# remit0/SpeechRecognitionProject

Hardware: AMD Instinct MI355X
Metric: utterances/sec (1 s @16 kHz) MFCC+CNN-BiGRU train step (higher is better)
Workload: dtype fp32; 1 GPU; cfg2 mfcc_bgru: on-device MFCC[39x51] + 2-layer BiGRU(512) + FC, CE, backward, Adam (full training.py step), per-GPU batch 256; model=mfcc_bgru, global_batch=256, clip_samples=16000, parallelism=dp1, step_execution=HIP graph replay of the whole step, sync_bn=False

## Files before the change

include/srk.h:

```cpp
#ifndef SRK_H_
#define SRK_H_

#include <stdint.h>

#define SRK_ABI_VERSION 3

#ifdef __cplusplus
extern "C" {
#endif

enum srk_status {
  SRK_OK = 0,
  SRK_ERR_INVALID = -1,
  SRK_ERR_HIP = -2,
  SRK_ERR_INTERNAL = -3,
  SRK_ERR_TIMEOUT = -4,
};

int srk_version(void);
const char* srk_source_stamp(void);
const char* srk_last_error(void);
int srk_init(int device);
int64_t srk_scratch_generation(void);
int srk_prof_enable(int on);
// ... 24 lines not shown
                  const int64_t* file_idx, const int64_t* offset, const double* gain,
                  int64_t n_clips, float* out, void* stream);

int srk_spec_noise_fwd(const int16_t* pcm, const int16_t* bank, int64_t n_files, int64_t bank_len,
                       const int64_t* file_idx, const int64_t* offset, const double* gain, int64_t n_clips,
                       float* out, int transposed, void* stream);

int srk_softmax_ensemble(const float* logits, int64_t K, int64_t B, int64_t C, float* probs_cat, float* mean,
                         int64_t* pred, void* stream);

enum { SRK_WAV_ERR_OPEN = -1, SRK_WAV_ERR_FORMAT = -2, SRK_WAV_ERR_UNSUPPORTED = -3 };
int srk_wav_read_batch(const char* const* paths, int64_t n, int16_t* out, int64_t* lengths, int n_threads);

enum { SRK_AUG_NONE = 0, SRK_AUG_SPEED = 1, SRK_AUG_SHIFT = 2, SRK_AUG_NOISE = 3, SRK_AUG_NOISE_SNR = 4,
       SRK_AUG_SILENCE = 5, SRK_AUG_PITCH = 6  };
int srk_augment(const int16_t* pcm, int64_t n_clips, const int16_t* bank, int64_t bank_len, const int32_t* op,
                const int64_t* iparam, const int64_t* noise_pos, const double* dparam, uint64_t seed, float* out,
                void* stream);

int64_t srk_pitch_workspace_bytes(int64_t n_shift);
int srk_pitch_shift(const int16_t* pcm, int64_t n_clips, const int32_t* clip_idx, const int32_t* level_idx,
                    int64_t n_shift, float* out, void* workspace, int64_t workspace_bytes, void* stream);

int srk_gemm_f32(int trans_a, int trans_b, int64_t M, int64_t N, int64_t K, float alpha, const float* A,
                 int64_t lda, const float* B, int64_t ldb, float beta, float* C, int64_t ldc,
                 const float* bias, int bias_mode, void* stream);
int srk_gemm_rowsum_f32(int trans_a, int trans_b, int64_t M, int64_t N, int64_t K, float alpha, const float* A,
                        int64_t lda, const float* B, int64_t ldb, float beta, float* C, int64_t ldc,
                        float* rowsum, void* stream);
int srk_gemm_16(int trans_a, int trans_b, int64_t M, int64_t N, int64_t K, float alpha, const uint16_t* A,
                int64_t lda, const uint16_t* B, int64_t ldb, float beta, float* C, int64_t ldc,
                const float* bias, int bias_mode, void* stream);
int srk_gemm_16_batched(int trans_a, int trans_b, int64_t M, int64_t N, int64_t K, float alpha,
                        const uint16_t* A, int64_t lda, int64_t sA, const uint16_t* B, int64_t ldb,
                        int64_t sB, float beta, float* C, int64_t ldc, int64_t sC, int batch, void* stream);
int srk_colsum_f32(const float* X, int64_t M, int64_t N, int64_t ldx, float* out, float beta, void* stream);

int64_t srk_gru_workspace_floats(int64_t B, int64_t T, int64_t in, int64_t H, int backward);
int srk_gru_layer_fwd(const float* x, int64_t B, int64_t T, int64_t in, int64_t H, const float* w_ih,
                      const float* w_hh, const float* b_ih, const float* b_hh, float* y, float* ws,
                      void* stream);
int srk_gru_layer_bwd(const float* x, int64_t B, int64_t T, int64_t in, int64_t H, const float* w_ih,
                      const float* w_hh, const float* y, const float* ws_fwd, const float* dy, float* dx,
                      float* dw_ih, float* dw_hh, float* db_ih, float* db_hh, int accumulate, float* ws,
                      void* stream);
int64_t srk_gru_y16_offset(int64_t B, int64_t T, int64_t in, int64_t H);
int srk_gru_layer_fwd_x16(const float* x, const void* x16, int64_t B, int64_t T, int64_t in, int64_t H,
                          const float* w_ih, const float* w_hh, const float* b_ih, const float* b_hh, float* y,
                          float* ws, void* stream);
int srk_gru_layer_bwd_x16(const float* x, const void* x16, int64_t B, int64_t T, int64_t in, int64_t H,
                          const float* w_ih, const float* w_hh, const float* y, const float* ws_fwd, const float* dy,
                          float* dx, float* dw_ih, float* dw_hh, float* db_ih, float* db_hh, int accumulate,
                          float* ws, void* stream);

int64_t srk_conv2d_workspace_floats(int64_t Ci, int64_t Co, int64_t KH, int64_t KW);
int srk_conv2d_nhwc_fwd(const float* x, int64_t N, int64_t H, int64_t W, int64_t Ci, const float* w,
                        const float* bias, int64_t Co, int64_t KH, int64_t KW, int64_t ph, int64_t pw, int64_t sh,
                        int64_t sw, float* y, float* ws, void* stream);
int srk_conv2d_nhwc_bwd(const float* x, int64_t N, int64_t H, int64_t W, int64_t Ci, const float* w, int64_t Co,
                        int64_t KH, int64_t KW, int64_t ph, int64_t pw, int64_t sh, int64_t sw, const float* dy,
                        float* dx, float* dw, float* db, float* ws, void* stream);
int srk_conv2d_nhwc_fwd16(const float* x, int64_t N, int64_t H, int64_t W, int64_t Ci, const float* w,
                          const float* bias, int64_t Co, int64_t KH, int64_t KW, int64_t ph, int64_t pw, int64_t sh,
                          int64_t sw, float* y, float* ws, void* x16, int* x16_written, void* stream);
int srk_conv2d_nhwc_bwd16(const float* x, int64_t N, int64_t H, int64_t W, int64_t Ci, const float* w, int64_t Co,
                          int64_t KH, int64_t KW, int64_t ph, int64_t pw, int64_t sh, int64_t sw, const float* dy,
                          float* dx, float* dw, float* db, float* ws, const void* x16, void* stream);
int srk_conv2d_nhwc_bwd16_dy16(const float* x, int64_t N, int64_t H, int64_t W, int64_t Ci, const float* w,
                               int64_t Co, int64_t KH, int64_t KW, int64_t ph, int64_t pw, int64_t sh, int64_t sw,
                               const float* dy, const void* dy16, float* dx, float* dw, float* db, float* ws,
                               const void* x16, void* stream);
int srk_conv2d_nhwc_bwd16_acc(const float* x, int64_t N, int64_t H, int64_t W, int64_t Ci, const float* w,
                              int64_t Co, int64_t KH, int64_t KW, int64_t ph, int64_t pw, int64_t sh, int64_t sw,
                              const float* dy, const void* dy16, float* dx, float* dw, float* db, float* ws,
                              const void* x16, int dw_accumulate, void* stream);
int srk_conv1d_nlc_dil_fwd(const float* x, int64_t N, int64_t L, int64_t Ci, const float* w, const float* bias,
                           int64_t Co, int64_t K, int64_t pad, int64_t dil, float* y, float* ws,
                           void* x16, int* x16_written, void* stream);
int srk_conv1d_nlc_dil_bwd(const float* x, int64_t N, int64_t L, int64_t Ci, const float* w, int64_t Co, int64_t K,
                           int64_t pad, int64_t dil, const float* dy, const void* dy16, float* dx, float* dw,
                           float* db, float* ws, const void* x16, int dw_accumulate, void* stream);
int srk_conv2d_nhwc_fwd_pool(const float* x, int64_t N, int64_t H, int64_t W, int64_t Ci, const float* w,
                             const float* bias, int64_t Co, int64_t KH, int64_t KW, int64_t ph, int64_t pw,
                             int64_t pool_w, float* y, uint8_t* argmax, float* ws, void* x16, int* x16_written,
                             void* stream);
int srk_conv2d_nhwc_bwd_pool(const float* x, int64_t N, int64_t H, int64_t W, int64_t Ci, const float* w, int64_t Co,
                             int64_t KH, int64_t KW, int64_t ph, int64_t pw, int64_t pool_w, const float* dy_pooled,
                             const uint8_t* argmax, float* dx, float* dw, float* db, float* ws, const void* x16,
                             void* stream);
int64_t srk_conv1_pool_workspace_floats(int64_t Co, int64_t KH, int64_t KW);
int srk_conv1_pool_fwd(const float* x, int64_t N, int64_t H, int64_t W, const float* w, const float* bias,
                       int64_t Co, int64_t KH, int64_t KW, int64_t ph, int64_t pw, int64_t pool, float* y,
                       uint8_t* argmax, void* stream);
int srk_conv1_pool_fwd16(const float* x, int64_t N, int64_t H, int64_t W, const float* w, const float* bias,
                         int64_t Co, int64_t KH, int64_t KW, int64_t ph, int64_t pw, int64_t pool, float* y,
                         uint8_t* argmax, void* y16, int* y16_written, void* stream);
int srk_conv1_pool_wgrad(const float* x, int64_t N, int64_t H, int64_t W, int64_t Co, int64_t KH, int64_t KW,
                         int64_t ph, int64_t pw, int64_t pool, const float* dy, const uint8_t* argmax, float* dw,
                         float* db, float* ws, void* stream);
int srk_conv1_pool_dgrad(const float* w, int64_t N, int64_t H, int64_t W, int64_t Co, int64_t KH, int64_t KW,
                         int64_t ph, int64_t pw, int64_t pool, const float* dy, const uint8_t* argmax, float* dx,
                         void* stream);
int srk_maxpool_nhwc_fwd(const float* x, int64_t N, int64_t H, int64_t W, int64_t C, int64_t kh, int64_t kw,
                         float* y, void* stream);
int srk_maxpool_nhwc_bwd(const float* x, const float* dy, int64_t N, int64_t H, int64_t W, int64_t C, int64_t kh,
                         int64_t kw, float* dx, void* stream);
// ... 88 lines not shown
```

speechrecognitionproject_amd/_lib.py:

```python
import ctypes
import os
import re

import torch

_HERE = os.path.dirname(os.path.abspath(__file__))
LIB_PATH = os.environ.get("SRK_LIB") or os.path.join(_HERE, "libsrk.so")
HEADER = os.path.join(os.path.dirname(_HERE), "include", "srk.h")
ABI_VERSION = 3

_P = ctypes.c_void_p
_I64 = ctypes.c_int64
_I = ctypes.c_int
_F = ctypes.c_float
_D = ctypes.c_double

_SIGS = {
    "srk_version": [],
    "srk_last_error": [],
    "srk_init": [_I],
    "srk_prof_enable": [_I],
    "srk_prof_read": [ctypes.c_char_p, ctypes.POINTER(ctypes.c_int64), ctypes.POINTER(ctypes.c_double),
                      ctypes.POINTER(ctypes.c_double)],
    "srk_prof_kernels": [ctypes.c_char_p, _I64, ctypes.POINTER(ctypes.c_int64)],
    "srk_source_stamp": [],
    "srk_diag_acc_store": [_P, _I64, _I, _P],
    "srk_diag_tr16_read": [_P, _I64, _P, _P],
    "srk_set_option": [ctypes.c_char_p, _I64],
    "srk_spin_timeouts": [],
    "srk_scratch_generation": [],
    "srk_gru_audit_words": [_I64, _I, _I, ctypes.POINTER(ctypes.c_int64), ctypes.POINTER(ctypes.c_int64),
                            ctypes.POINTER(ctypes.c_int64)],
    "srk_health_check": [_I],
    "srk_health_reset": [],
    "srk_fbank_fwd": [_P, _I64, _P, _P],
    "srk_mfcc_fwd": [_P, _I64, _P, _I, _P],
    "srk_spec_fwd": [_P, _I64, _P, _I, _P],
    "srk_fbank_fwd_i16": [_P, _I64, _P, _P],
    "srk_mfcc_fwd_i16": [_P, _I64, _P, _I, _P],
    "srk_spec_fwd_i16": [_P, _I64, _P, _I, _P],
    "srk_fbank_vtlp_fwd": [_P, _I64, _P, _P, _P],
    "srk_fbank_vtlp_fwd_i16": [_P, _I64, _P, _P, _P],
    "srk_vtlp_bins": [_D, ctypes.POINTER(ctypes.c_int32)],
    "srk_uniform_f64_state": [_P, _D, _D, _I64, _P, _P],
    "srk_noise_mix": [_P, _P, _I64, _I64, _P, _P, _P, _I64, _P, _P],
    "srk_spec_noise_fwd": [_P, _P, _I64, _I64, _P, _P, _P, _I64, _P, _I, _P],
    "srk_augment": [_P, _I64, _P, _I64, _P, _P, _P, _P, ctypes.c_uint64, _P, _P],
    "srk_pitch_workspace_bytes": [_I64],
    "srk_pitch_shift": [_P, _I64, _P, _P, _I64, _P, _P, _I64, _P],
    "srk_wav_read_batch": [ctypes.POINTER(ctypes.c_char_p), _I64, _P, _P, _I],
    "srk_softmax_ensemble": [_P, _I64, _I64, _I64, _P, _P, _P, _P],
    "srk_gemm_f32": [_I, _I, _I64, _I64, _I64, _F, _P, _I64, _P, _I64, _F, _P, _I64, _P, _I, _P],
    "srk_gemm_rowsum_f32": [_I, _I, _I64, _I64, _I64, _F, _P, _I64, _P, _I64, _F, _P, _I64, _P, _P],
    "srk_gemm_16": [_I, _I, _I64, _I64, _I64, _F, _P, _I64, _P, _I64, _F, _P, _I64, _P, _I, _P],
    "srk_gemm_16_batched": [_I, _I, _I64, _I64, _I64, _F, _P, _I64, _I64, _P, _I64, _I64, _F, _P, _I64, _I64, _I, _P],
    "srk_colsum_f32": [_P, _I64, _I64, _I64, _P, _F, _P],
    "srk_gru_workspace_floats": [_I64, _I64, _I64, _I64, _I],
    "srk_gru_layer_fwd": [_P, _I64, _I64, _I64, _I64, _P, _P, _P, _P, _P, _P, _P],
    "srk_gru_layer_bwd": [_P, _I64, _I64, _I64, _I64, _P, _P, _P, _P, _P, _P, _P, _P, _P, _P, _I, _P, _P],
    "srk_gru_y16_offset": [_I64, _I64, _I64, _I64],
    "srk_gru_layer_fwd_x16": [_P, _P, _I64, _I64, _I64, _I64, _P, _P, _P, _P, _P, _P, _P],
    "srk_gru_layer_bwd_x16": [_P, _P, _I64, _I64, _I64, _I64, _P, _P, _P, _P, _P, _P, _P, _P, _P, _P, _I, _P, _P],
    "srk_conv2d_workspace_floats": [_I64, _I64, _I64, _I64],
    "srk_conv2d_nhwc_fwd": [_P, _I64, _I64, _I64, _I64, _P, _P, _I64, _I64, _I64, _I64, _I64, _I64, _I64, _P, _P,
                            _P],
    "srk_conv2d_nhwc_bwd": [_P, _I64, _I64, _I64, _I64, _P, _I64, _I64, _I64, _I64, _I64, _I64, _I64, _P, _P, _P,
                            _P, _P, _P],
    "srk_conv2d_nhwc_fwd16": [_P, _I64, _I64, _I64, _I64, _P, _P, _I64, _I64, _I64, _I64, _I64, _I64, _I64, _P, _P,
                              _P, ctypes.POINTER(_I), _P],
    "srk_conv2d_nhwc_bwd16": [_P, _I64, _I64, _I64, _I64, _P, _I64, _I64, _I64, _I64, _I64, _I64, _I64, _P, _P, _P,
                              _P, _P, _P, _P],
    "srk_conv2d_nhwc_bwd16_dy16": [_P, _I64, _I64, _I64, _I64, _P, _I64, _I64, _I64, _I64, _I64, _I64, _I64, _P, _P,
                                   _P, _P, _P, _P, _P, _P],
    "srk_conv2d_nhwc_bwd16_acc": [_P, _I64, _I64, _I64, _I64, _P, _I64, _I64, _I64, _I64, _I64, _I64, _I64, _P, _P,
                                  _P, _P, _P, _P, _P, _I, _P],
    "srk_conv1d_nlc_dil_fwd": [_P, _I64, _I64, _I64, _P, _P, _I64, _I64, _I64, _I64, _P, _P, _P, ctypes.POINTER(_I), _P],
    "srk_conv1d_nlc_dil_bwd": [_P, _I64, _I64, _I64, _P, _I64, _I64, _I64, _I64, _P, _P, _P, _P, _P, _P, _P, _I, _P],
    "srk_conv2d_nhwc_fwd_pool": [_P, _I64, _I64, _I64, _I64, _P, _P, _I64, _I64, _I64, _I64, _I64, _I64, _P, _P, _P,
                                 _P, ctypes.POINTER(_I), _P],
    "srk_conv2d_nhwc_bwd_pool": [_P, _I64, _I64, _I64, _I64, _P, _I64, _I64, _I64, _I64, _I64, _I64, _P, _P, _P, _P,
                                 _P, _P, _P, _P],
    "srk_conv1_pool_workspace_floats": [_I64, _I64, _I64],
    "srk_conv1_pool_fwd": [_P, _I64, _I64, _I64, _P, _P, _I64, _I64, _I64, _I64, _I64, _I64, _P, _P, _P],
    "srk_conv1_pool_fwd16": [_P, _I64, _I64, _I64, _P, _P, _I64, _I64, _I64, _I64, _I64, _I64, _P, _P, _P, _P, _P],
    "srk_conv1_pool_wgrad": [_P, _I64, _I64, _I64, _I64, _I64, _I64, _I64, _I64, _I64, _P, _P, _P, _P, _P, _P],
    "srk_conv1_pool_dgrad": [_P, _I64, _I64, _I64, _I64, _I64, _I64, _I64, _I64, _I64, _P, _P, _P, _P],
    "srk_maxpool_nhwc_fwd": [_P, _I64, _I64, _I64, _I64, _I64, _I64, _P, _P],
    "srk_maxpool_nhwc_bwd": [_P, _P, _I64, _I64, _I64, _I64, _I64, _I64, _P, _P],
    "srk_batchnorm_fwd": [_P, _I64, _I64, _P, _P, _F, _F, _I, _P, _P, _P, _I, _P, _P, _P, _P],
    "srk_batchnorm_bwd": [_P, _P, _P, _I64, _I64, _P, _P, _P, _I, _I, _P, _P, _P, _P, _P],
    "srk_batchnorm_fwd16": [_P, _I64, _I64, _P, _P, _F, _F, _I, _P, _P, _P, _I, _P, _P, ctypes.POINTER(_I), _P, _P,
                            _P],
    "srk_batchnorm_bwd16": [_P, _P, _P, _I64, _I64, _P, _P, _P, _I, _I, _P, _P, ctypes.POINTER(_I), _P, _P, _P, _P],
    "srk_batchnorm_bwd16_acc": [_P, _P, _P, _I64, _I64, _P, _P, _P, _I, _I, _P, _P, ctypes.POINTER(_I), _P, _P, _P,
                                _P, _P, _P],
    "srk_batchnorm_fwd16_mask": [_P, _I64, _I64, _P, _P, _F, _F, _I, _P, _P, _P, _I, _P, _P, ctypes.POINTER(_I), _P,
                                 _P, _P, _P],
    "srk_batchnorm_bwd16_mask": [_P, _P, _P, _P, _I64, _I64, _P, _P, _P, _I, _I, _P, _P, ctypes.POINTER(_I), _P, _P,
                                 _P, _P, _P, _P],
    "srk_batchnorm_stats": [_P, _I64, _I64, _P, _P],
    "srk_batchnorm_combine": [_P, _I, _I64, _F, _F, _P, _P, _P, _P, _P, _P],
    "srk_batchnorm_apply": [_P, _I64, _I64, _P, _P, _P, _P, _P, _I, _P, _P],
    "srk_batchnorm_bwd_reduce": [_P, _P, _P, _I64, _I64, _P, _P, _I, _P, _P],
    "srk_batchnorm_bwd_dx": [_P, _P, _P, _I64, _I64, _P, _P, _P, _P, _P, _I, _P, _P, _P],
    "srk_cross_entropy": [_P, _P, _I64, _I64, _P, _P, _P, _P],
    "srk_adam_step": [_P, _P, _P, _P, _I64, _F, _F, _F, _F, _I64, _F, _P],
    "srk_dropout_fwd": [_P, _I64, _F, ctypes.c_uint64, _P, _P, _P],
    "srk_dropout_fwd_state": [_P, _I64, _F, _P, _P, _P, _P],
    "srk_adam_step_state": [_P, _P, _P, _P, _I64, _F, _F, _F, _P, _F, _P],
    "srk_grad_scaler_init": [_P, _F, _F, _F, _I, _P],
    "srk_adam_step_scaled": [_P, _P, _P, _P, _I64, _F, _F, _F, _P, _F, _P, _P],
    "srk_dropout_apply": [_P, _P, _I64, _F, _P, _P],
    "srk_attn_pool_fwd": [_P, _P, _I64, _I64, _I64, _F, _P, _P, _P],
    "srk_attn_pool_bwd": [_P, _P, _P, _P, _I64, _I64, _I64, _F, _P, _P, _P],
    "srk_pcen_workspace_floats": [_I64, _I64, _I64],
    "srk_pcen_fwd": [_P, _P, _I64, _I64, _I64, _F, _F, _P, _P, _P],
    "srk_pcen_bwd": [_P, _P, _P, _P, _I64, _I64, _I64, _F, _F, _P, _P, _P, _P],
    "srk_dwconv2d_workspace_floats": [_I64] * 10,
    "srk_dwconv2d_nhwc_fwd": [_P, _I64, _I64, _I64, _I64, _P, _P, _I64, _I64, _I64, _I64, _I64, _I64, _P, _P],
    "srk_dwconv2d_nhwc_bwd": [_P, _I64, _I64, _I64, _I64, _P, _I64, _I64, _I64, _I64, _I64, _I64, _P, _P, _P, _P, _P,
                              _I, _P],
    "srk_avgpool_nhwc_fwd": [_P, _I64, _I64, _I64, _P, _P],
    "srk_avgpool_nhwc_bwd": [_P, _I64, _I64, _I64, _P, _P],
}
_RESTYPE = {"srk_last_error": ctypes.c_char_p, "srk_spin_timeouts": ctypes.c_int64, "srk_scratch_generation": ctypes.c_int64, "srk_gru_workspace_floats": ctypes.c_int64, "srk_gru_y16_offset": ctypes.c_int64,
            "srk_conv2d_workspace_floats": ctypes.c_int64, "srk_conv1_pool_workspace_floats": ctypes.c_int64,
            "srk_pitch_workspace_bytes": ctypes.c_int64, "srk_source_stamp": ctypes.c_char_p,
            "srk_pcen_workspace_floats": ctypes.c_int64, "srk_dwconv2d_workspace_floats": ctypes.c_int64}


class SrkError(RuntimeError):
    pass


_lib = None


def lib():
    global _lib
    if _lib is None:
        if not os.path.exists(LIB_PATH):
            raise SrkError("libsrk.so is not built (%s); run `python -m speechrecognitionproject_amd.build`" % LIB_PATH)
        L = ctypes.CDLL(LIB_PATH)
        for name, args in _SIGS.items():
            fn = getattr(L, name)
            fn.argtypes = args
            fn.restype = _RESTYPE.get(name, ctypes.c_int)
        v = L.srk_version()
        if v != ABI_VERSION:
            raise SrkError("libsrk.so ABI version %d != expected %d (rebuild)" % (v, ABI_VERSION))
        _lib = L
        for item in filter(None, os.environ.get("SRK_OPTIONS", "").split(",")):
            name, _, val = item.partition("=")
            call("srk_set_option", name.strip().encode(), int(val))
            _options[name.strip()] = int(val)
    return _lib


def source_stamp():
    return lib().srk_source_stamp().decode()


def call(name, *args):
    rc = getattr(lib(), name)(*args)
    if rc != 0:
        msg = lib().srk_last_error().decode(errors="replace")
        raise SrkError("%s failed (status %d): %s" % (name, rc, msg))
    return rc


def prof_enable(on):
    call("srk_prof_enable", 1 if on else 0)


def prof_read(name):
    n = ctypes.c_int64(0)
    ms = ctypes.c_double(0.0)
    w = ctypes.c_double(0.0)
# ... 91 lines not shown
```

speechrecognitionproject_amd/csrc/gemm.h:

```cpp
#pragma once
#include "srk_internal.h"

namespace srk {

struct GemmDesc {
  int64_t M = 0, N = 0, K = 0;
  const float* A = nullptr; int64_t lda = 0; bool ta = false;
  const float* B = nullptr; int64_t ldb = 0; bool tb = false;
  float* C = nullptr; int64_t ldc = 0;
  float alpha = 1.f, beta = 0.f;
  const float* bias = nullptr; int bias_mode = 0;
  int batch = 1; int64_t sA = 0, sB = 0, sC = 0;
  float* rowsum = nullptr; float rowsum_beta = 0.f;
  int64_t sRS = 0;
  int prec = -1;
  const uint16_t* A16 = nullptr;
  const uint16_t* B16 = nullptr;
};

int gemm_f32(const GemmDesc& d, hipStream_t stream);

bool gemm_f32_batched_rowsum_ok(const GemmDesc& d);

int colsum_f32(const float* X, int64_t M, int64_t N, int64_t ldx, float* out, float beta, hipStream_t stream);

}
```

speechrecognitionproject_amd/csrc/gemm.hip:

```cpp
#include <algorithm>
#include <cstdlib>
#include <mutex>
#include <type_traits>

#include "gemm.h"
#include "mfma_tile.h"

namespace srk {
namespace {

using namespace tile;

struct KernelArgs {
  GemmDesc d;
  int tiles_m, tiles_n;
  int tiles;
  int nblk;
  int group_m;
  int remap;
  int64_t kchunk;
  float* partial;
  float* rs_partial;
  int sk_wgs;
  int sk_ki;
// ... 1085 lines not shown
template <int RND, bool TA>
__global__ __launch_bounds__(256) void skinny_k_kernel(GemmDesc d) {
  const int64_t m = blockIdx.y, n = (int64_t)blockIdx.x * 256 + threadIdx.x;
  const int64_t nc = n < d.N ? n : d.N - 1;
  float av[16], bv[16];
#pragma unroll
  for (int k = 0; k < 16; ++k) {
    const bool ok = k < d.K;
    av[k] = ok ? (TA ? d.A[k * d.lda + m] : d.A[m * d.lda + k]) : 0.f;
    bv[k] = ok ? d.B[k * d.ldb + nc] : 0.f;
  }
  float acc = 0.f, rs = 0.f;
#pragma unroll
  for (int k = 0; k < 16; ++k) {
    rs += av[k];
    acc = fmaf(rnd16<RND>(av[k]), rnd16<RND>(bv[k]), acc);
  }
  if (n < d.N) skinny_store(d, m, n, acc);
  if (d.rowsum && blockIdx.x == 0 && threadIdx.x == 0)
    d.rowsum[m] = d.rowsum_beta != 0.f ? d.rowsum_beta * d.rowsum[m] + rs : rs;
}

inline double gemm_bytes(const GemmDesc& d, int esz) {
  const double c = (double)d.M * (double)d.N * 4.0 * (d.beta != 0.f ? 2.0 : 1.0);
  return ((double)d.M * (double)d.K * esz + (double)d.K * (double)d.N * esz + c) * (double)d.batch;
}

template <int RND>
int launch_skinny_rnd(const GemmDesc& d, int kind, hipStream_t s) {
  ProfScope prof(RND == 0 ? "gemm_f32" : RND == 1 ? "gemm_bf16" : "gemm_f16", s,
                 2.0 * (double)d.M * (double)d.N * (double)d.K);
  prof.bytes(gemm_bytes(d, 4));
  const char* kn = kind == 0 ? "skinny_n" : kind == 1 ? "skinny_m" : "skinny_k";
  prof.detail("%s_kernel<%c%c> %lldx%lldx%lld", kn, d.ta ? 'T' : 'N', d.tb ? 'T' : 'N', (long long)d.M,
              (long long)d.N, (long long)d.K);
  if (kind == 0) {
    const dim3 grid((unsigned)d.M);
    if (d.tb) hipLaunchKernelGGL((skinny_n_kernel<RND, true>), grid, dim3(256), 0, s, d);
    else hipLaunchKernelGGL((skinny_n_kernel<RND, false>), grid, dim3(256), 0, s, d);
  } else if (kind == 1) {
    const dim3 grid((unsigned)((d.N + 63) / 64));
    if (d.ta) hipLaunchKernelGGL((skinny_m_kernel<RND, true>), grid, dim3(1024), 0, s, d);
    else hipLaunchKernelGGL((skinny_m_kernel<RND, false>), grid, dim3(1024), 0, s, d);
  } else {
    const dim3 grid((unsigned)((d.N + 255) / 256), (unsigned)d.M);
    if (d.ta) hipLaunchKernelGGL((skinny_k_kernel<RND, true>), grid, dim3(256), 0, s, d);
    else hipLaunchKernelGGL((skinny_k_kernel<RND, false>), grid, dim3(256), 0, s, d);
  }
  SRK_CHECK_HIP(hipGetLastError());
  return SRK_OK;
}

int skinny_kind(const GemmDesc& d) {
  if (!g_opt_gemm_skinny || d.batch != 1 || d.A16 || d.B16 || d.K <= 0) return -1;
  if (d.N <= 16 && !d.ta && d.M <= 65535 * 16 && d.M * d.K <= (int64_t)1 << 24) return 0;
  if (d.M <= 16 && !d.tb && d.K <= 1024 && d.N * d.K <= (int64_t)1 << 24) return 1;
  if (d.K <= 16 && !d.tb && d.M <= 65535 && d.M * d.N <= (int64_t)1 << 24) return 2;
  return -1;
}

constexpr int kP32BK = 16;
template <bool KC>
struct P32Half {
  static constexpr int FLOATS = 128 * kP32BK;
  __device__ static __forceinline__ v4f frag(const float* img, int r0, int kb, int lane) {
    const int row = r0 + (lane & 31), h = lane >> 5;
    if (KC) return *reinterpret_cast<const v4f*>(img + row * kP32BK + (((2 * kb + h) ^ ((row >> 2) & 3)) << 2));
    const float* q = img + (8 * kb + 4 * h) * 128 + row;
    return v4f{q[0], q[128], q[256], q[384]};
  }
  __device__ static __forceinline__ void src(int piece, int lane, int64_t r0, int64_t rows, int64_t ld, unsigned& voff,
                                             int& kk, bool& row_ok) {
    const int p = piece * 64 + lane;
    if (KC) {
      const int row = p >> 2, kc = (p & 3) ^ ((row >> 2) & 3);
      voff = (unsigned)(((r0 + row) * ld + kc * 4) * 4);
      kk = kc * 4;
      row_ok = r0 + row < rows;
    } else {
      const int k = p >> 5, u = p & 31;
      voff = (unsigned)((k * ld + r0 + u * 4) * 4);
      kk = k;
      row_ok = r0 + u * 4 < rows;
    }
  }
  __device__ static __forceinline__ int64_t kstep_bytes(int64_t ld) { return KC ? 4 : 4 * ld; }
};

template <bool TA, bool TB>
__global__ __launch_bounds__(512, 1) void gemm_p32_kernel(KernelArgs ka) {
  constexpr int BK = kP32BK, NST = 4;
  constexpr bool AKC = !TA, BKC = TB;
  using HA = P32Half<AKC>;
  using HB = P32Half<BKC>;
  constexpr int HALF = HA::FLOATS;
  constexpr int STAGE = 4 * HALF;
  __shared__ __attribute__((aligned(1024))) float smem[NST * STAGE];
  typedef __attribute__((address_space(3))) void* lds_ptr;
  auto bar = [] {
    asm volatile("" ::: "memory");
    __builtin_amdgcn_s_barrier();
    asm volatile("" ::: "memory");
  };
  const GemmDesc& d = ka.d;
  const int tid = threadIdx.x, lane = tid & 63, wave = tid >> 6, grp = wave >> 2, wc = wave & 3;
  const bool sk = ka.sk_wgs > 0;
  int64_t sk_it = 0, sk_end = 0;
// ... 284 lines not shown
    if (part_out) part_out[(int64_t)blockIdx.y * N + col] = t;
    else out[col] = beta != 0.f ? beta * out[col] + t : t;
  }
}

struct Scratch {
  float* p = nullptr;
  size_t floats = 0;
};
Scratch g_scratch[64];
std::mutex g_scratch_mu;

int get_scratch(size_t floats, float** out) {
  int dev = 0;
  SRK_CHECK_HIP(hipGetDevice(&dev));
  SRK_REQUIRE(dev >= 0 && dev < 64, SRK_ERR_INVALID, "device out of range");
  std::lock_guard<std::mutex> lk(g_scratch_mu);
  Scratch& s = g_scratch[dev];
  if (s.floats < floats) {
    if (s.p) {
      SRK_CHECK_HIP(hipDeviceSynchronize());
      SRK_CHECK_HIP(hipFree(s.p));
      s.p = nullptr;
    }
    const size_t want = floats + floats / 4;
    SRK_CHECK_HIP(hipMalloc(reinterpret_cast<void**>(&s.p), want * sizeof(float)));
    g_scratch_gen.fetch_add(1);
    s.floats = want;
  }
  *out = s.p;
  return SRK_OK;
}

int env_int(const char* name, int dflt) {
  const char* v = getenv(name);
  return v && *v ? atoi(v) : dflt;
}

int plan_launch(const GemmDesc& d, int BM, int BN, int BK, int per_cu, KernelArgs& ka, int* splits_out,
                bool allow_split = true, bool split_batched = false) {
  const int64_t tm = (d.M + BM - 1) / BM, tn = (d.N + BN - 1) / BN;
  SRK_REQUIRE(tm * tn <= (INT32_MAX >> 5) && d.batch <= 65535, SRK_ERR_INVALID, "gemm: grid too large");
  static const int remap = env_int("SRK_GEMM_REMAP", 1);
  const int64_t slots = (int64_t)kCUs * per_cu;
  ka = KernelArgs{};
  ka.d = d;
  ka.tiles_m = (int)tm;
  ka.tiles_n = (int)tn;
  ka.tiles = (int)(tm * tn);
  static const int group_env = env_int("SRK_GROUP_M", 0);
  ka.group_m = group_env > 0 ? group_env
                             : std::max(1, (int)std::lround(std::sqrt(32.0 * per_cu * BN / (double)BM)));
  ka.remap = remap;
  const bool can_split = allow_split && (d.batch == 1 || split_batched);
  int splits = can_split ? choose_splits(tm * tn * d.batch, d.K, BK, slots, 16) : 1;
  static const int splits_env = env_int("SRK_GEMM_SPLITS", 0);
  if (splits_env > 0 && d.batch == 1 && d.K >= (int64_t)splits_env * 4 * BK) splits = splits_env;
  ka.kchunk = splits > 1 ? ((d.K + splits - 1) / splits + BK - 1) / BK * BK : std::max<int64_t>(d.K, 1);
  if (splits > 1) splits = (int)((d.K + ka.kchunk - 1) / ka.kchunk);
  ka.nblk = ka.tiles * splits;
  if (splits > 1) {
    float* scratch = nullptr;
    const size_t need = (size_t)d.batch * splits * (d.M * d.N + (d.rowsum ? d.M : 0));
    if (int rc = get_scratch(need, &scratch)) return rc;
    ka.partial = scratch;
    ka.rs_partial = d.rowsum ? scratch + (size_t)d.batch * splits * d.M * d.N : nullptr;
  }
  *splits_out = splits;
  return SRK_OK;
}

int finish_splits(const GemmDesc& d, const KernelArgs& ka, int splits, hipStream_t s) {
  SRK_CHECK_HIP(hipGetLastError());
  if (splits > 1) {
    const int64_t n = d.M * d.N;
    const bool vec4 = d.N % 4 == 0 && d.ldc % 4 == 0 && (uintptr_t)d.C % 16 == 0 && d.sC % 4 == 0 &&
                      (d.bias_mode != 1 || (uintptr_t)d.bias % 16 == 0);
    if (vec4)
      hipLaunchKernelGGL(splitk_reduce4_kernel, dim3((unsigned)((n / 4 + 255) / 256), (unsigned)d.batch), dim3(256), 0,
                         s, d, ka.partial, splits);
    else
      hipLaunchKernelGGL(splitk_reduce_kernel, dim3((unsigned)((n + 255) / 256), (unsigned)d.batch), dim3(256), 0, s, d,
                         ka.partial, splits);
    if (d.rowsum)
      hipLaunchKernelGGL(rowsum_reduce_kernel, dim3((unsigned)((d.M + 255) / 256), (unsigned)d.batch), dim3(256), 0, s,
                         d.rowsum, d.rowsum_beta, ka.rs_partial, d.M, splits, d.sRS);
    SRK_CHECK_HIP(hipGetLastError());
  }
  return SRK_OK;
}

template <bool TA, bool TB, int BM, int BN, int BK>
int launch(const GemmDesc& d, hipStream_t s, bool vec) {
  constexpr int lds = 2 * 4 * (Img<!TA, BM, BK>::FLOATS + Img<TB, BN, BK>::FLOATS);
  constexpr int per_cu0 = (160 * 1024) / lds < 8 ? (160 * 1024) / lds : 8;
  constexpr int per_cu = per_cu0 > 0 ? per_cu0 : 1;
  KernelArgs ka;
  int splits = 1;
  if (int rc = plan_launch(d, BM, BN, BK, per_cu, ka, &splits)) return rc;
  ProfScope prof("gemm_f32", s, 2.0 * (double)d.M * (double)d.N * (double)d.K * d.batch);
  prof.bytes(gemm_bytes(d, 4));
  static const int waves_env = env_int("SRK_GEMM_WAVES", 0);
  const int waves = BM == 256 ? 8 : (waves_env ? waves_env : ((!TA && TB) ? 4 : 8));
  prof.detail("gemm_f32_kernel<%c%c,%dx%d,%dw> %lldx%lldx%lld b%lld s%d", TA ? 'T' : 'N', TB ? 'T' : 'N', BM, BN, waves,
              (long long)d.M, (long long)d.N, (long long)d.K, (long long)d.batch, splits);
  const dim3 grid((unsigned)ka.nblk, 1, (unsigned)d.batch);
  static const int glds_env = env_int("SRK_GEMM_GLDS", 1);
  const bool gl = vec && glds_env != 0;
// ... 50 lines not shown
    case 4: return launch_lp_cfg<TA, TB, 256, 128, 8, 2>(d, s, vec, f16);
    case 5: return launch_lp_cfg<TA, TB, 128, 128, 8, 2>(d, s, vec, f16);
    default: return launch_lp_cfg<TA, TB, 128, 128, 4, 1>(d, s, vec, f16);
  }
}

template <bool TA, bool TB, int BM, int BN, int NW>
int launch_h16_cfg(const GemmDesc& d, hipStream_t s, bool f16) {
  constexpr int per_cu = h16_per_cu<TA, TB, BM, BN>();
  KernelArgs ka;
  int splits = 1;
  if (int rc = plan_launch(d, BM, BN, kLpBK, per_cu, ka, &splits)) return rc;
  ProfScope prof(f16 ? "gemm_f16" : "gemm_bf16", s, 2.0 * (double)d.M * (double)d.N * (double)d.K);
  prof.bytes(gemm_bytes(d, 2));
  prof.detail("gemm_h16_kernel<%c%c,%dx%d> %lldx%lldx%lld s%d", TA ? 'T' : 'N', TB ? 'T' : 'N', BM, BN, (long long)d.M,
              (long long)d.N, (long long)d.K, splits);
  const dim3 grid((unsigned)ka.nblk), block(NW * 64);
  if (f16) hipLaunchKernelGGL((gemm_h16_kernel<TA, TB, BM, BN, NW, true>), grid, block, 0, s, ka);
  else hipLaunchKernelGGL((gemm_h16_kernel<TA, TB, BM, BN, NW, false>), grid, block, 0, s, ka);
  return finish_splits(d, ka, splits, s);
}

template <bool TA, bool TB>
int launch_g16(const GemmDesc& d, hipStream_t s, bool f16) {
  KernelArgs ka;
  int splits = 1;
  const int64_t tiles = ((d.M + 255) / 256) * ((d.N + 255) / 256) * d.batch;
  if (int rc = plan_launch(d, 256, 256, kG16BK, 1, ka, &splits, tiles * 2 < kCUs, true)) return rc;
  ProfScope prof(f16 ? "gemm_f16" : "gemm_bf16", s, 2.0 * (double)d.M * (double)d.N * (double)d.K * d.batch);
  prof.bytes(gemm_bytes(d, 2));
  prof.detail("gemm_g16_kernel<%c%c> %lldx%lldx%lld b%d s%d", TA ? 'T' : 'N', TB ? 'T' : 'N', (long long)d.M,
              (long long)d.N, (long long)d.K, d.batch, splits);
  const dim3 grid((unsigned)ka.nblk, (unsigned)d.batch), block(512);
  if (f16) hipLaunchKernelGGL((gemm_g16_kernel<TA, TB, true>), grid, block, 0, s, ka);
  else hipLaunchKernelGGL((gemm_g16_kernel<TA, TB, false>), grid, block, 0, s, ka);
  return finish_splits(d, ka, splits, s);
}

template <bool TA, bool TB>
int launch_h16(const GemmDesc& d, hipStream_t s, bool f16) {
  static const int cfg_env = env_int("SRK_H16_CFG", 0);
  const int kern = g_opt_gemm16_kernel ? g_opt_gemm16_kernel : (d.M >= 1024 && d.N >= 256 ? 2 : 1);
  if (kern == 2 || cfg_env == 5 || d.batch > 1) return launch_g16<TA, TB>(d, s, f16);
  const int cfg = cfg_env ? cfg_env : d.M < 1024 ? 1 : (TA != TB && d.N >= 256) ? 4 : 3;
  if (cfg == 3) return launch_h16_cfg<TA, TB, 256, 128, 8>(d, s, f16);
  if (cfg == 4) return launch_h16_cfg<TA, TB, 256, 256, 8>(d, s, f16);
  return launch_h16_cfg<TA, TB, 128, 128, 4>(d, s, f16);
}

template <bool TA, bool TB>
int launch_p32(const GemmDesc& d, hipStream_t s) {
  KernelArgs ka;
  int splits = 1;
  const int64_t tiles = ((d.M + 255) / 256) * ((d.N + 255) / 256) * d.batch;
  const int64_t ki = (d.K + kP32BK - 1) / kP32BK;
  const bool streamk = g_opt_gemm_streamk && d.batch == 1 && !d.rowsum && tiles < kCUs && tiles * 2 >= kCUs && ki >= 32;
  if (int rc = plan_launch(d, 256, 256, kP32BK, 1, ka, &splits, !streamk && tiles * 2 < kCUs, true)) return rc;
  if (streamk) {
    ka.sk_wgs = kCUs;
    ka.sk_ki = (int)ki;
    ka.nblk = kCUs;
    if (int rc = get_scratch((size_t)3 * d.M * d.N, &ka.sk_slab)) return rc;
  }
  ProfScope prof("gemm_f32", s, 2.0 * (double)d.M * (double)d.N * (double)d.K * d.batch);
  prof.bytes(gemm_bytes(d, 4));
  prof.detail("gemm_p32_kernel<%c%c> %lldx%lldx%lld b%d s%d%s", TA ? 'T' : 'N', TB ? 'T' : 'N', (long long)d.M,
              (long long)d.N, (long long)d.K, d.batch, splits, streamk ? " streamk" : "");
  hipLaunchKernelGGL((gemm_p32_kernel<TA, TB>), dim3((unsigned)ka.nblk, (unsigned)d.batch), dim3(512), 0, s, ka);
  if (streamk) hipLaunchKernelGGL(sk_fixup_kernel, dim3((unsigned)ka.tiles * kSkFixupSlices), dim3(256), 0, s, ka);
  return finish_splits(d, ka, splits, s);
}

template <bool TA, bool TB>
int dispatch_tile(const GemmDesc& d, hipStream_t s, bool vec) {
  const int prec = d.prec >= 0 ? d.prec : matmul_prec();
  if (prec != kPrecF32) return launch_lp<TA, TB>(d, s, vec, prec == kPrecF16);
  const double ext_a = (double)(d.ta ? d.K : d.M) * d.lda * 4, ext_b = (double)(d.tb ? d.N : d.K) * d.ldb * 4;
  const bool p32_ok = vec && ext_a < 2147483000.0 && ext_b < 2147483000.0;
  const int kern32 = g_opt_gemm32_kernel ? g_opt_gemm32_kernel
                                         : (!TB && ((d.M >= 2048 && d.N >= 1024) || d.batch > 1) ? 2 : 1);
  SRK_REQUIRE(!d.rowsum || d.batch == 1 || (p32_ok && kern32 == 2), SRK_ERR_INVALID,
              "gemm: batched row sums need the fp32 ping-pong kernel (16-B operand rows)");
  if (p32_ok && kern32 == 2) return launch_p32<TA, TB>(d, s);
  static const int tile_env = env_int("SRK_GEMM_TILE", 0);
  const int64_t t256 = ((d.M + 255) / 256) * ((d.N + 127) / 128) * d.batch;
  const bool big = tile_env ? tile_env == 256 : (d.M >= 2048 && d.N >= 128 && d.K >= 256 && (t256 >= 512 || d.K >= 4096));
  if (big) return launch<TA, TB, 256, 128, 32>(d, s, vec);
  const int64_t big_tiles = ((d.M + 127) / 128) * ((d.N + 127) / 128) * d.batch;
  if (d.M > 64 && d.N > 64 && (big_tiles >= 64 || d.K >= 2048)) return launch<TA, TB, 128, 128, 32>(d, s, vec);
  return launch<TA, TB, 64, 64, 32>(d, s, vec);
}

}

bool gemm_f32_batched_rowsum_ok(const GemmDesc& d) {
  const int prec = d.prec >= 0 ? d.prec : matmul_prec();
  if (prec != kPrecF32 || d.A16 || d.B16 || d.tb || g_opt_gemm32_kernel == 1) return false;
  const bool kc_operand = !d.ta || d.tb;
  const bool vec = (d.lda % 4 == 0) && ((uintptr_t)d.A % 16 == 0) && (d.sA % 4 == 0) && (d.ldb % 4 == 0) &&
                   ((uintptr_t)d.B % 16 == 0) && (d.sB % 4 == 0) && (!kc_operand || d.K % 4 == 0) &&
                   (!d.ta || d.M % 4 == 0) && (d.tb || d.N % 4 == 0);
  const double ext_a = (double)(d.ta ? d.K : d.M) * d.lda * 4, ext_b = (double)(d.tb ? d.N : d.K) * d.ldb * 4;
  const double span_a = ext_a + (double)(d.batch - 1) * d.sA * 4, span_b = ext_b + (double)(d.batch - 1) * d.sB * 4;
  return vec && span_a < 2147483000.0 && span_b < 2147483000.0;
}

int gemm_f32(const GemmDesc& d, hipStream_t s) {
  SRK_REQUIRE(d.M >= 0 && d.N >= 0 && d.K >= 0 && d.batch >= 1, SRK_ERR_INVALID, "gemm: bad shape");
  if (d.M == 0 || d.N == 0) return SRK_OK;
  if (d.A16 || d.B16) {
    const int prec = d.prec >= 0 ? d.prec : matmul_prec();
    SRK_REQUIRE(d.A16 && d.B16 && d.C && prec != kPrecF32 && !d.rowsum && (d.batch == 1 || d.bias_mode == 0),
                SRK_ERR_INVALID,
                "gemm: 16-bit operands need both A16 / B16, a 16-bit precision and no row sums (no bias when batched)");
    SRK_REQUIRE(d.batch == 1 || (d.sA % 8 == 0 && d.sB % 8 == 0 && d.sC % 4 == 0), SRK_ERR_INVALID,
                "gemm: batched 16-bit operands need 8-element strides");
    const double ext_a = (double)(d.ta ? d.K : d.M) * d.lda * 2, ext_b = (double)(d.tb ? d.N : d.K) * d.ldb * 2;
    SRK_REQUIRE((uintptr_t)d.A16 % 16 == 0 && (uintptr_t)d.B16 % 16 == 0 && d.lda % 8 == 0 && d.ldb % 8 == 0 &&
                    ((d.ta && d.M % 8 == 0) || (!d.ta && d.K % 8 == 0)) &&
                    ((d.tb && d.K % 8 == 0) || (!d.tb && d.N % 8 == 0)) && ext_a < 2147483648.0 &&
                    ext_b < 2147483648.0,
                SRK_ERR_INVALID, "gemm: 16-bit operands need 16-B aligned rows of 8-element multiples");
    SRK_REQUIRE(d.K > 0, SRK_ERR_INVALID, "gemm: 16-bit operands need K > 0");
    const bool f16 = prec == kPrecF16;
    if (!d.ta && !d.tb) return launch_h16<false, false>(d, s, f16);
    if (!d.ta && d.tb) return launch_h16<false, true>(d, s, f16);
    if (d.ta && !d.tb) return launch_h16<true, false>(d, s, f16);
    return launch_h16<true, true>(d, s, f16);
  }
  SRK_REQUIRE(d.C && (d.K == 0 || (d.A && d.B)), SRK_ERR_INVALID, "gemm: null operand");
  SRK_REQUIRE(d.bias_mode == 0 || d.bias, SRK_ERR_INVALID, "gemm: bias_mode without bias");
  if (const int kind = skinny_kind(d); kind >= 0) {
    const int prec = d.prec >= 0 ? d.prec : matmul_prec();
// ... 122 lines not shown
```

speechrecognitionproject_amd/csrc/gru.hip:

```cpp
#include <algorithm>
#include <mutex>

#include "gemm.h"
#include "gru_internal.h"

namespace srk {
namespace {

constexpr int kRows = 64;
constexpr int kUnits = 16;
constexpr int kBK = 128;
constexpr int kPitch = kBK + 4;

struct GruArgs {
  int B, T, H, in;
  int G, S;
  const float* y_in;
  float* y;
  const float* gi;
  const float* w_hh;
  const float* b_hh;
  float* gates;
  const float* dy;
  float* dgi;
  float* dgh;
  float* dgh_edge;
  float* dhz;
};

__device__ __forceinline__ float sigmoidf_(float x) { return 1.0f / (1.0f + expf(-x)); }

typedef float v4f __attribute__((ext_vector_type(4)));
__device__ __forceinline__ v4f ld4(const float* p) { return *reinterpret_cast<const v4f*>(p); }
__device__ __forceinline__ void st4(float* p, v4f v) { *reinterpret_cast<v4f*>(p) = v; }

__device__ __forceinline__ void map_block(const GruArgs& a, int& dir, int& group, int& slice) {
  const int nwg = 2 * a.G * a.S;
  const int b = blockIdx.x, xcd = b & 7, q = nwg >> 3, r = nwg & 7;
  const int wgid = (xcd < r ? xcd * (q + 1) : r * (q + 1) + (xcd - r) * q) + (b >> 3);
  const int pair = wgid / a.S;
  slice = wgid % a.S;
  dir = pair / a.G;
  group = pair % a.G;
}

__global__ __launch_bounds__(256) void gru_fwd_step_kernel(GruArgs a, int step) {
  constexpr int WR = 3 * kUnits;
  constexpr int VA = kRows * kBK / 4 / 256;
  constexpr int VW = WR * kBK / 4 / 256;
  __shared__ __attribute__((aligned(16))) float smem[2 * (kRows + WR) * kPitch];
  const int tid = threadIdx.x, lane = tid & 63, wave = tid >> 6;
  const int lr = lane & 15, lq = lane >> 4;
  int dir, group, slice;
  map_block(a, dir, group, slice);
  const int B = a.B, T = a.T, H = a.H;
  const int t = dir == 0 ? step : T - 1 - step;
  const int tprev = dir == 0 ? t - 1 : t + 1;
  const int b0 = group * kRows, j0 = slice * kUnits;
  const float* __restrict__ W = a.w_hh + (size_t)dir * 3 * H * H;

  typedef float f32x4 __attribute__((ext_vector_type(4)));
  f32x4 acc[3];
#pragma unroll
  for (int g = 0; g < 3; ++g) acc[g] = f32x4{0.f, 0.f, 0.f, 0.f};

  if (step > 0) {
    v4f ra[VA], rw[VW];
    auto load = [&](int k0) {
#pragma unroll
      for (int i = 0; i < VA; ++i) {
        const int v = tid + i * 256, row = v / (kBK / 4), kq = (v % (kBK / 4)) * 4;
        const int b = b0 + row;
        const v4f x = ld4(a.y_in + ((size_t)(b < B ? b : B - 1) * T + tprev) * 2 * H + dir * H + k0 + kq);
        ra[i] = b < B ? x : v4f{0.f, 0.f, 0.f, 0.f};
      }
#pragma unroll
      for (int i = 0; i < VW; ++i) {
        const int v = tid + i * 256, c = v / (kBK / 4), kq = (v % (kBK / 4)) * 4;
        const int g = c / kUnits, jj = c % kUnits;
        rw[i] = ld4(W + (size_t)(g * H + j0 + jj) * H + k0 + kq);
      }
    };
    auto store = [&](int buf) {
// ... 121 lines not shown
    for (int kt = 0; kt < nk; ++kt) {
      const int cur = kt & 1;
      if (kt + 1 < nk) load((kt + 1) * kBK);
      const float* As = smem + cur * (kRows + kUnits) * kPitch;
      const float* Ws = As + kRows * kPitch;
#pragma unroll
      for (int kb = 0; kb < kBK; kb += 16) {
        const v4f av = ld4(As + (wave * 16 + lr) * kPitch + kb + 4 * lq);
        const v4f wv = ld4(Ws + lr * kPitch + kb + 4 * lq);
        acc[0] = __builtin_amdgcn_mfma_f32_16x16x4f32(av.x, wv.x, acc[0], 0, 0, 0);
        acc[1] = __builtin_amdgcn_mfma_f32_16x16x4f32(av.y, wv.y, acc[1], 0, 0, 0);
        acc[0] = __builtin_amdgcn_mfma_f32_16x16x4f32(av.z, wv.z, acc[0], 0, 0, 0);
        acc[1] = __builtin_amdgcn_mfma_f32_16x16x4f32(av.w, wv.w, acc[1], 0, 0, 0);
      }
      asm volatile("" ::: "memory");
      __builtin_amdgcn_sched_barrier(0);
      if (kt + 1 < nk) store(cur ^ 1);
      __syncthreads();
    }
  }

  const int j = j0 + lr;
#pragma unroll
  for (int r = 0; r < 4; ++r) {
    const int b = b0 + wave * 16 + lq * 4 + r;
    if (b >= B) continue;
    float* dhz = a.dhz + ((size_t)dir * B + b) * H + j;
    float dh = a.dy[((size_t)b * T + t) * 2 * H + dir * H + j];
    if (step > 0) dh += (acc[0][r] + acc[1][r]) + *dhz;
    const float* gs = a.gates + (((size_t)dir * T + t) * B + b) * 4 * H;
    const float rg = gs[j], zg = gs[H + j], ng = gs[2 * H + j], ghn = gs[3 * H + j];
    const float hp = edge ? 0.f : a.y_in[((size_t)b * T + tprev) * 2 * H + dir * H + j];
    const float dn = dh * (1.0f - zg);
    const float daz = dh * (hp - ng) * zg * (1.0f - zg);
    const float dan = dn * (1.0f - ng * ng);
    const float dar = dan * ghn * rg * (1.0f - rg);
    float* dgi = a.dgi + ((size_t)b * T + t) * 6 * H + dir * 3 * H;
    dgi[j] = dar;
    dgi[H + j] = daz;
    dgi[2 * H + j] = dan;
    float* dg = edge ? a.dgh_edge + ((size_t)dir * B + b) * 3 * H
                     : a.dgh + (((size_t)dir * B + b) * T + t) * 3 * H;
    dg[j] = dar;
    dg[H + j] = daz;
    dg[2 * H + j] = dan * rg;
    if (edge) {
      float* z0 = a.dgh + (((size_t)dir * B + b) * T + t) * 3 * H;
      z0[j] = 0.f; z0[H + j] = 0.f; z0[2 * H + j] = 0.f;
    }
    *dhz = dh * zg;
  }
}

int check_dims(int64_t B, int64_t T, int64_t in, int64_t H) {
  SRK_REQUIRE(B > 0 && T > 0 && in > 0 && H > 0, SRK_ERR_INVALID, "gru: dims must be positive");
  SRK_REQUIRE(H % kBK == 0, SRK_ERR_INVALID, "gru: hidden size must be a multiple of 128");
  SRK_REQUIRE(B * T * 6 * H < ((int64_t)1 << 40), SRK_ERR_INVALID, "gru: problem too large");
  return SRK_OK;
}

__global__ void pad_cols_kernel(const float* __restrict__ src, int64_t rows, int cols, float* __restrict__ dst,
                                int colsp) {
  const int64_t i = (int64_t)blockIdx.x * blockDim.x + threadIdx.x;
  if (i >= rows * colsp) return;
  const int64_t r = i / colsp;
  const int c = (int)(i - r * colsp);
  dst[i] = c < cols ? src[r * cols + c] : 0.f;
}
__global__ void unpad_cols_kernel(const float* __restrict__ src, int64_t rows, int colsp, float* __restrict__ dst,
                                  int cols, int accumulate) {
  const int64_t i = (int64_t)blockIdx.x * blockDim.x + threadIdx.x;
  if (i >= rows * cols) return;
  const int64_t r = i / cols;
  const int c = (int)(i - r * cols);
  const float v = src[r * colsp + c];
  dst[i] = accumulate ? dst[i] + v : v;
}
template <bool F16>
__global__ void to16_kernel(const float* __restrict__ src, int64_t rows, int cols, uint16_t* __restrict__ dst,
                            int colsp) {
  const int64_t i = (int64_t)blockIdx.x * blockDim.x + threadIdx.x;
  if (i >= rows * colsp) return;
  const int64_t r = i / colsp;
  const int c = (int)(i - r * colsp);
  const float v = c < cols ? src[r * cols + c] : 0.f;
  if (F16) {
    const _Float16 h = (_Float16)v;
    dst[i] = __builtin_bit_cast(uint16_t, h);
  } else {
    const __bf16 h = (__bf16)v;
    dst[i] = __builtin_bit_cast(uint16_t, h);
  }
}
template <bool F16>
__global__ void to16_vec8_kernel(const float* __restrict__ src, int64_t n8, uint16_t* __restrict__ dst) {
  const int64_t i = (int64_t)blockIdx.x * blockDim.x + threadIdx.x;
  if (i >= n8) return;
  typedef float f4 __attribute__((ext_vector_type(4)));
  typedef unsigned u4 __attribute__((ext_vector_type(4)));
  typedef __attribute__((ext_vector_type(8))) typename std::conditional<F16, _Float16, __bf16>::type e8;
  const f4 a = *reinterpret_cast<const f4*>(src + 8 * i), b = *reinterpret_cast<const f4*>(src + 8 * i + 4);
  const e8 h = __builtin_convertvector((__attribute__((ext_vector_type(8))) float){a.x, a.y, a.z, a.w, b.x, b.y, b.z, b.w}, e8);
  *reinterpret_cast<u4*>(dst + 8 * i) = __builtin_bit_cast(u4, h);
}

int to16(const float* src, int64_t rows, int64_t cols, uint16_t* dst, int64_t colsp, hipStream_t s) {
// ... 114 lines not shown
static int64_t fwd_xbuf_off(int64_t B, int64_t T, int64_t H) { return (B * T * 6 * H + 2 * T * B * 4 * H + 63) / 64 * 64; }
static int64_t bwd_xbuf_off(int64_t B, int64_t T, int64_t H) {
  return (B * T * 6 * H + 2 * B * T * 3 * H + 2 * B * 3 * H + 2 * B * H + 63) / 64 * 64;
}
static int64_t xbuf_rows(int64_t B) { return std::min<int64_t>((B + 63) / 64 * 64, 512); }
static int64_t fwd_counter_off(int64_t B, int64_t T, int64_t H) {
  return fwd_xbuf_off(B, T, H) + 2 * srk::kHandoffSlots * xbuf_rows(B) * H;
}
static int64_t bwd_counter_off(int64_t B, int64_t T, int64_t H) {
  return bwd_xbuf_off(B, T, H) + 6 * srk::kHandoffSlots * xbuf_rows(B) * H;
}

static int64_t pad_off(int64_t B, int64_t T, int64_t H, int backward) {
  return ((backward ? bwd_counter_off(B, T, H) : fwd_counter_off(B, T, H)) + srk::kCounterFloats + 63) / 64 * 64;
}

static int64_t pad_end(int64_t B, int64_t T, int64_t in, int64_t H, int backward) {
  int64_t e = pad_off(B, T, H, backward) + 64;
  if (srk::padded_in(in)) {
    const int64_t in4 = srk::pad4(in);
    e += (backward ? 2 * 6 * H * in4 + B * T * in4 : B * T * in4 + 6 * H * in4) + 64;
  }
  return (e + 63) / 64 * 64;
}
static int64_t up64(int64_t v) { return (v + 63) / 64 * 64; }
static int64_t in8_of(int64_t in) { return (in + 7) / 8 * 8; }
static int64_t h16_floats(int64_t B, int64_t T, int64_t in, int64_t H, int backward) {
  const int64_t in8 = in8_of(in), BT = B * T;
  if (!backward) return up64(BT * in8 / 2 + 1) + up64(6 * H * in8 / 2 + 1) + up64(BT * 2 * H / 2 + 1);
  const int64_t chunks = (B + 255) / 256;
  return up64(chunks * 8 * 2 * 4 * H) + (in8 != in ? up64(6 * H * in8) + up64(BT * in8) : 0);
}
static bool use_h16(int64_t B, int64_t T, int64_t in, int64_t H) {
  return srk::matmul_prec() != srk::kPrecF32 && srk::g_opt_gru_persistent &&
         srk::gru_persistent_supported(B, T, H, false) && srk::gru_persistent_supported(B, T, H, true) &&
         (double)B * T * 6 * H * 2 < 2147483647.0 && (double)B * T * in8_of(in) * 2 < 2147483647.0;
}

int64_t srk_gru_workspace_floats(int64_t B, int64_t T, int64_t in, int64_t H, int backward) {
  return pad_end(B, T, in, H, backward) + (H == 512 ? h16_floats(B, T, in, H, backward) + 64 : 0);
}

int srk_gru_layer_fwd(const float* x, int64_t B, int64_t T, int64_t in, int64_t H, const float* w_ih,
                      const float* w_hh, const float* b_ih, const float* b_hh, float* y, float* ws, void* stream) {
  return srk_gru_layer_fwd_x16(x, nullptr, B, T, in, H, w_ih, w_hh, b_ih, b_hh, y, ws, stream);
}

int64_t srk_gru_y16_offset(int64_t B, int64_t T, int64_t in, int64_t H) {
  if (srk::check_dims(B, T, in, H) || H != 512 || !use_h16(B, T, in, H)) return -1;
  const int64_t in8 = in8_of(in), BT = B * T;
  return pad_end(B, T, in, H, 0) + up64(BT * in8 / 2 + 1) + up64(6 * H * in8 / 2 + 1);
}

int srk_gru_layer_fwd_x16(const float* x, const void* x16_in, int64_t B, int64_t T, int64_t in, int64_t H,
                          const float* w_ih, const float* w_hh, const float* b_ih, const float* b_hh, float* y,
                          float* ws, void* stream) {
  SRK_API_BEGIN
  if (int rc = srk::check_dims(B, T, in, H)) return rc;
  SRK_REQUIRE(x && w_ih && w_hh && b_ih && b_hh && y && ws, SRK_ERR_INVALID, "gru_fwd: null pointer");
  hipStream_t s = srk::as_stream(stream);
  float* gi = ws;
  float* gates = ws + B * T * 6 * H;
  uint16_t* y16 = nullptr;
  if (use_h16(B, T, in, H)) {
    const int64_t in8 = in8_of(in), BT = B * T;
    uint16_t* x16 = reinterpret_cast<uint16_t*>(ws + pad_end(B, T, in, H, 0));
    uint16_t* w16 = x16 + 2 * up64(BT * in8 / 2 + 1);
    y16 = w16 + 2 * up64(6 * H * in8 / 2 + 1);
    SRK_REQUIRE(!x16_in || (in8 == in && reinterpret_cast<uintptr_t>(x16_in) % 16 == 0), SRK_ERR_INVALID,
                "gru_fwd: a ready 16-bit x needs in % 8 == 0 and 16-B alignment");
    if (x16_in) x16 = const_cast<uint16_t*>(static_cast<const uint16_t*>(x16_in));
    else if (int rc = srk::to16(x, BT, in, x16, in8, s)) return rc;
    const bool fuse = in <= srk::kFusedIn;
    if (!fuse) {
      if (int rc = srk::to16(w_ih, 6 * H, in, w16, in8, s)) return rc;
      GemmDesc g;
      g.M = BT; g.N = 6 * H; g.K = in8;
      g.A16 = x16; g.lda = in8;
      g.B16 = w16; g.ldb = in8; g.tb = true;
      g.C = gi; g.ldc = 6 * H;
      g.bias = b_ih; g.bias_mode = 1;
      if (int rc = srk::gemm_f32(g, s)) return rc;
    }
    srk::GruPArgs p{};
    p.B = (int)B; p.T = (int)T; p.H = (int)H;
    p.gi = gi; p.w_hh = w_hh; p.b_hh = b_hh; p.y = y; p.gates = gates; p.y16 = y16;
    if (fuse) { p.x_in = x; p.w_ih = w_ih; p.b_ih = b_ih; p.in = (int)in; }
    p.xbuf = ws + fwd_xbuf_off(B, T, H);
    p.counters = reinterpret_cast<unsigned*>(ws + fwd_counter_off(B, T, H));
    return srk::gru_persistent_launch(p, false, s);
  }
  const float* xa = x;
  const float* wa = w_ih;
  int64_t ink = in;
  if (srk::padded_in(in)) {
    ink = srk::pad4(in);
    float* xp = ws + pad_off(B, T, H, 0);
    float* wp = xp + B * T * ink;
    if (int rc = srk::pad_cols(x, B * T, in, xp, s)) return rc;
    if (int rc = srk::pad_cols(w_ih, 6 * H, in, wp, s)) return rc;
    xa = xp;
    wa = wp;
  }
  const bool persistent = srk::g_opt_gru_persistent && srk::gru_persistent_supported(B, T, H, false) &&
                          srk::gru_persistent_supported(B, T, H, true);
  const bool fuse = persistent && in <= srk::kFusedIn;
  if (!fuse) {
    GemmDesc g;
    g.M = B * T; g.N = 6 * H; g.K = ink;
    g.A = xa; g.lda = ink;
    g.B = wa; g.ldb = ink; g.tb = true;
    g.C = gi; g.ldc = 6 * H;
    g.bias = b_ih; g.bias_mode = 1;
    if (int rc = srk::gemm_f32(g, s)) return rc;
  }
  if (persistent) {
    srk::GruPArgs p{};
    p.B = (int)B; p.T = (int)T; p.H = (int)H;
    p.gi = gi; p.w_hh = w_hh; p.b_hh = b_hh; p.y = y; p.gates = gates;
    if (fuse) { p.x_in = x; p.w_ih = w_ih; p.b_ih = b_ih; p.in = (int)in; }
    p.xbuf = ws + fwd_xbuf_off(B, T, H);
    p.counters = reinterpret_cast<unsigned*>(ws + fwd_counter_off(B, T, H));
    return srk::gru_persistent_launch(p, false, s);
  }
  srk::GruArgs a{};
  a.B = (int)B; a.T = (int)T; a.H = (int)H; a.in = (int)in;
  a.y_in = y; a.y = y; a.gi = gi; a.w_hh = w_hh; a.b_hh = b_hh; a.gates = gates;
  a.G = (int)((B + srk::kRows - 1) / srk::kRows);
  a.S = (int)(H / srk::kUnits);
  const dim3 grid((unsigned)(2 * a.G * a.S));
  for (int step = 0; step < T; ++step) {
    srk::ProfScope prof("gru_fwd_step", s, step > 0 ? 2.0 * 2.0 * (double)B * 3 * H * H : 0.0);
    hipLaunchKernelGGL(srk::gru_fwd_step_kernel, grid, dim3(256), 0, s, a, step);
  }
  SRK_CHECK_HIP(hipGetLastError());
  return SRK_OK;
  SRK_API_END
}

int srk_gru_layer_bwd(const float* x, int64_t B, int64_t T, int64_t in, int64_t H, const float* w_ih,
                      const float* w_hh, const float* y, const float* ws_fwd, const float* dy, float* dx,
                      float* dw_ih, float* dw_hh, float* db_ih, float* db_hh, int accumulate, float* ws,
                      void* stream) {
  return srk_gru_layer_bwd_x16(x, nullptr, B, T, in, H, w_ih, w_hh, y, ws_fwd, dy, dx, dw_ih, dw_hh, db_ih, db_hh,
                               accumulate, ws, stream);
}

int srk_gru_layer_bwd_x16(const float* x, const void* x16_in, int64_t B, int64_t T, int64_t in, int64_t H,
                          const float* w_ih, const float* w_hh, const float* y, const float* ws_fwd, const float* dy,
                          float* dx, float* dw_ih, float* dw_hh, float* db_ih, float* db_hh, int accumulate,
                          float* ws, void* stream) {
  SRK_API_BEGIN
  if (int rc = srk::check_dims(B, T, in, H)) return rc;
  SRK_REQUIRE(x && w_ih && w_hh && y && ws_fwd && dy && dw_ih && dw_hh && db_ih && db_hh && ws, SRK_ERR_INVALID,
              "gru_bwd: null pointer");
  hipStream_t s = srk::as_stream(stream);
  const int64_t BT = B * T;
  if (use_h16(B, T, in, H)) {
    const int64_t in8 = in8_of(in);
    const uint16_t* x16 = reinterpret_cast<const uint16_t*>(ws_fwd + pad_end(B, T, in, H, 0));
    const uint16_t* w16 = x16 + 2 * up64(BT * in8 / 2 + 1);
    const uint16_t* y16 = w16 + 2 * up64(6 * H * in8 / 2 + 1);
    if (x16_in) x16 = static_cast<const uint16_t*>(x16_in);
    uint16_t* dgi16 = reinterpret_cast<uint16_t*>(ws);
    uint16_t* dgh16 = dgi16 + BT * 6 * H;
    float* part = ws + pad_end(B, T, in, H, 1);
    const int64_t chunks = (B + 255) / 256;
    float* dwpad = part + up64(chunks * 8 * 2 * 4 * H);
    float* dxpad = dwpad + up64(6 * H * in8);
    srk::GruPArgs p{};
    p.B = (int)B; p.T = (int)T; p.H = (int)H;
    p.w_hh = w_hh; p.y_in = y; p.gates = const_cast<float*>(ws_fwd + BT * 6 * H); p.dy = dy;
    p.dgi16 = dgi16; p.dgh16 = dgh16; p.dbias = part;
    p.xbuf = ws + bwd_xbuf_off(B, T, H);
    p.counters = reinterpret_cast<unsigned*>(ws + bwd_counter_off(B, T, H));
    int rc;
    const int dw_parts = srk::gru_dwhh_fused_parts(B, T);
    if (dw_parts) {
      if ((rc = srk::gru_scratch((size_t)dw_parts * 2 * 3 * H * H, &p.dw_part))) return rc;
      p.y16_in = y16;
    }
    if ((rc = srk::gru_persistent_launch(p, true, s))) return rc;
    const int prows = srk::gru_bias_part_rows(B);
    if (dw_parts) {
      const int64_t per_dir = 3 * H * H, n4 = 2 * per_dir / 4;
      const int dw_blocks = (int)((n4 + 255) / 256);
      srk::ProfScope prof("gru_dwhh_reduce", s, 4.0 * (dw_parts + 2) * 2 * per_dir);
      hipLaunchKernelGGL(srk::dwhh_dbias_reduce_kernel, dim3((unsigned)(dw_blocks + (6 * H + 255) / 256)), dim3(256),
                         0, s, p.dw_part, dw_parts, (int)B, per_dir, dw_hh, (int)accumulate, dw_blocks, part,
                         (int)(chunks * (256 / prows)), (int)H, prows, db_ih, db_hh);
    } else {
      hipLaunchKernelGGL(srk::dbias_reduce_kernel, dim3((unsigned)((6 * H + 255) / 256)), dim3(256), 0, s, part,
                         (int)(chunks * (256 / prows)), (int)B, (int)H, prows, db_ih, db_hh, accumulate);
    }
    SRK_CHECK_HIP(hipGetLastError());
    const float beta = accumulate ? 1.f : 0.f;
    {
      GemmDesc g;
      g.M = 6 * H; g.N = in8; g.K = BT;
      g.A16 = dgi16; g.lda = 6 * H; g.ta = true;
      g.B16 = x16; g.ldb = in8;
      g.C = in8 == in ? dw_ih : dwpad; g.ldc = in8; g.beta = in8 == in ? beta : 0.f;
      if ((rc = srk::gemm_f32(g, s))) return rc;
      if (in8 != in) {
        const int64_t n = 6 * H * in;
        hipLaunchKernelGGL(srk::unpad_cols_kernel, dim3((unsigned)((n + 255) / 256)), dim3(256), 0, s, dwpad, 6 * H,
                           (int)in8, dw_ih, (int)in, (int)accumulate);
        SRK_CHECK_HIP(hipGetLastError());
      }
    }
    {
      GemmDesc g;
      g.M = 3 * H; g.N = H; g.K = BT - 1;
      g.ta = true; g.lda = 3 * H; g.ldb = 2 * H;
      g.A16 = dgh16 + 3 * H;
      g.B16 = y16;
      g.C = dw_hh; g.ldc = H; g.beta = beta;
      g.batch = 2; g.sA = BT * 3 * H - 3 * H; g.sB = 3 * H; g.sC = 3 * H * H;
      if (dw_parts) {
      } else if (g.K > 0 && srk::g_opt_gru_dwhh_batched) {
        if ((rc = srk::gemm_f32(g, s))) return rc;
      } else if (g.K > 0) {
        g.batch = 1;
        for (int dir = 0; dir < 2; ++dir, g.A16 += g.sA, g.B16 += g.sB, g.C += g.sC)
          if ((rc = srk::gemm_f32(g, s))) return rc;
      } else if (!accumulate) {
        SRK_CHECK_HIP(hipMemsetAsync(g.C, 0, sizeof(float) * 2 * 3 * H * H, s));
      }
    }
    if (dx) {
      if (in <= srk::kFusedIn) {
        if ((rc = srk::to16(w_ih, 6 * H, in, const_cast<uint16_t*>(w16), in8, s))) return rc;
      }
      GemmDesc g;
      g.M = BT; g.N = in8; g.K = 6 * H;
      g.A16 = dgi16; g.lda = 6 * H;
      g.B16 = w16; g.ldb = in8;
      g.C = in8 == in ? dx : dxpad; g.ldc = in8;
      if ((rc = srk::gemm_f32(g, s))) return rc;
      if (in8 != in) {
        const int64_t n = BT * in;
        hipLaunchKernelGGL(srk::unpad_cols_kernel, dim3((unsigned)((n + 255) / 256)), dim3(256), 0, s, dxpad, BT,
                           (int)in8, dx, (int)in, 0);
        SRK_CHECK_HIP(hipGetLastError());
      }
    }
    return SRK_OK;
  }
  float* dgi = ws;
  float* dgh = dgi + BT * 6 * H;
  float* dgh_edge = dgh + 2 * BT * 3 * H;
  float* dhz = dgh_edge + 2 * B * 3 * H;
  srk::GruArgs a{};
  a.B = (int)B; a.T = (int)T; a.H = (int)H; a.in = (int)in;
  a.y_in = y; a.w_hh = w_hh; a.gates = const_cast<float*>(ws_fwd + BT * 6 * H);
  a.dy = dy; a.dgi = dgi; a.dgh = dgh; a.dgh_edge = dgh_edge; a.dhz = dhz;
  a.G = (int)((B + srk::kRows - 1) / srk::kRows);
  a.S = (int)(H / srk::kUnits);
  if (srk::g_opt_gru_persistent && srk::gru_persistent_supported(B, T, H, false) &&
      srk::gru_persistent_supported(B, T, H, true)) {
    srk::GruPArgs p{};
    p.B = (int)B; p.T = (int)T; p.H = (int)H;
    p.w_hh = w_hh; p.y_in = y; p.gates = a.gates; p.dy = dy; p.dgi = dgi; p.dgh = dgh; p.dgh_edge = dgh_edge;
    p.xbuf = ws + bwd_xbuf_off(B, T, H);
    p.counters = reinterpret_cast<unsigned*>(ws + bwd_counter_off(B, T, H));
    if (int rc = srk::gru_persistent_launch(p, true, s)) return rc;
  } else {
  const dim3 grid((unsigned)(2 * a.G * a.S));
  for (int step = 0; step < T; ++step) {
    srk::ProfScope prof("gru_bwd_step", s, step > 0 ? 2.0 * 2.0 * (double)B * 3 * H * H : 0.0);
    hipLaunchKernelGGL(srk::gru_bwd_step_kernel, grid, dim3(256), 0, s, a, step);
  }
  SRK_CHECK_HIP(hipGetLastError());
  }

  int rc;
  const float beta = accumulate ? 1.f : 0.f;
  const bool pad = srk::padded_in(in);
  const int64_t in4 = srk::pad4(in);
  float* wpad = pad ? ws + pad_off(B, T, H, 1) : nullptr;
  float* dwpad = pad ? wpad + 6 * H * in4 : nullptr;
  float* dxpad = pad ? dwpad + 6 * H * in4 : nullptr;
  {
    GemmDesc g;
    g.M = 6 * H; g.N = pad ? in4 : in; g.K = BT;
    g.A = dgi; g.lda = 6 * H; g.ta = true;
    g.B = pad ? ws_fwd + pad_off(B, T, H, 0) : x; g.ldb = pad ? in4 : in;
    g.C = pad ? dwpad : dw_ih; g.ldc = pad ? in4 : in; g.beta = pad ? 0.f : beta;
    g.rowsum = db_ih; g.rowsum_beta = beta;
    if ((rc = srk::gemm_f32(g, s))) return rc;
    if (pad) {
      const int64_t n = 6 * H * in;
      hipLaunchKernelGGL(srk::unpad_cols_kernel, dim3((unsigned)((n + 255) / 256)), dim3(256), 0, s, dwpad, 6 * H,
                         (int)in4, dw_ih, (int)in, (int)accumulate);
      SRK_CHECK_HIP(hipGetLastError());
    }
  }
  {
    GemmDesc g;
    g.M = 3 * H; g.N = H; g.K = BT - 1;
    g.ta = true; g.lda = 3 * H; g.ldb = 2 * H;
    g.A = dgh + 3 * H;
    g.B = y;
    g.C = dw_hh; g.ldc = H; g.beta = beta;
    g.rowsum = db_hh; g.rowsum_beta = beta;
    g.batch = 2; g.sA = BT * 3 * H - 3 * H; g.sB = 3 * H; g.sC = 3 * H * H; g.sRS = 3 * H;
    const bool batched = srk::g_opt_gru_dwhh_batched && srk::gemm_f32_batched_rowsum_ok(g);
    if (g.K > 0 && batched) {
      if ((rc = srk::gemm_f32(g, s))) return rc;
    } else if (g.K > 0) {
      g.batch = 1;
      for (int dir = 0; dir < 2; ++dir, g.A += g.sA, g.B += g.sB, g.C += g.sC, g.rowsum += g.sRS)
        if ((rc = srk::gemm_f32(g, s))) return rc;
    } else if (!accumulate) {
      SRK_CHECK_HIP(hipMemsetAsync(dw_hh, 0, sizeof(float) * 2 * 3 * H * H, s));
      SRK_CHECK_HIP(hipMemsetAsync(db_hh, 0, sizeof(float) * 2 * 3 * H, s));
    }
    for (int dir = 0; dir < 2; ++dir)
      if ((rc = srk::colsum_f32(dgh_edge + (size_t)dir * B * 3 * H, B, 3 * H, 3 * H, db_hh + dir * 3 * H, 1.f, s)))
        return rc;
  }
  if (dx) {
    GemmDesc g;
    g.M = BT; g.N = pad ? in4 : in; g.K = 6 * H;
    g.A = dgi; g.lda = 6 * H;
    if (pad && (rc = srk::pad_cols(w_ih, 6 * H, in, wpad, s))) return rc;
    g.B = pad ? wpad : w_ih; g.ldb = pad ? in4 : in;
    g.C = pad ? dxpad : dx; g.ldc = pad ? in4 : in;
    if ((rc = srk::gemm_f32(g, s))) return rc;
    if (pad) {
      const int64_t n = BT * in;
      hipLaunchKernelGGL(srk::unpad_cols_kernel, dim3((unsigned)((n + 255) / 256)), dim3(256), 0, s, dxpad, BT,
                         (int)in4, dx, (int)in, 0);
      SRK_CHECK_HIP(hipGetLastError());
    }
  }
  return SRK_OK;
  SRK_API_END
}

}
```

speechrecognitionproject_amd/csrc/gru_internal.h:

```cpp
#pragma once
#include <algorithm>

#include "srk_internal.h"

namespace srk {

constexpr int kCounterFloats = 4096;
constexpr int kCensusOff = 4080;
__host__ __device__ constexpr int pw_counter(int dir, int G, int group) { return (dir * G + group) * 16; }
__host__ __device__ constexpr int pw_flag64(int dir, int G, int group, int slot) { return (dir * G + group) * 32 + slot; }
__host__ __device__ constexpr int pw_flag_lp2(int dir, int G, int group, int slot) { return (dir * G + group) * 16 + slot; }
__host__ __device__ constexpr int pw_flag_dc(int dir, int G, int group, int c, int rb, int slot) {
  return (((dir * G + group) * 2 + c) * 2 + rb) * 64 + slot;
}
constexpr int kHandoffSlots = 3;
constexpr int kFusedIn = 64;

struct GruPArgs {
  int B, T, H;
  int G;
  int b_begin, b_end;
  const float* gi;
  const float* w_hh;
  const float* b_hh;
  float* y;
  const float* y_in;
  float* gates;
  const float* dy;
  float* dgi;
  float* dgh;
  float* dgh_edge;
  float* xbuf;
  unsigned* counters;
  int flags;
  int xcd_local;
  uint16_t* y16;
  uint16_t* dgi16;
  uint16_t* dgh16;
  float* dbias;
  int chunk;
  const float* x_in;
  const float* w_ih;
  const float* b_ih;
  int in;
  unsigned long long* trace;
  unsigned* health;
  unsigned spin_limit;
  unsigned dc_offset;
  int fast_cell;
  int dc_prio;
  const uint16_t* y16_in;
  float* dw_part;
  int dw_mode;
};

size_t fwd_lds_bytes(int H);
size_t bwd_lds_bytes(int H);
int gru_persistent_supported(int64_t B, int64_t T, int64_t H, bool backward);
int gru_persistent_launch(GruPArgs a, bool backward, hipStream_t s);

extern int g_opt_gru_persistent;
extern unsigned long long* g_opt_gru_trace;
extern unsigned g_opt_gru_spin_limit;
extern int g_opt_gru_xcd_local;
extern int g_opt_gru_lp_wide;
extern int g_opt_gru_lp2;
extern int g_opt_gru_dc;
extern unsigned g_opt_gru_dc_offset;
extern int g_opt_gru_fast_cell;
extern int g_opt_gru_dc_prio;
int gru_bias_part_rows(int64_t B);
int gru_dwhh_fused_parts(int64_t B, int64_t T);
extern int g_opt_gru_dwhh_fused;
extern int g_opt_gru_fwd_worker;
int health_word(unsigned** host, unsigned** dev);

}
```

speechrecognitionproject_amd/csrc/gru_persistent.hip:

```cpp
#include <cstdlib>
#include <type_traits>
#include <mutex>
#include <utility>

#include "gru_internal.h"

namespace srk {

__device__ unsigned long long g_spin_timeouts = 0;

namespace {

typedef float v4f __attribute__((ext_vector_type(4)));
typedef unsigned v4u __attribute__((ext_vector_type(4)));
typedef float f32x4 __attribute__((ext_vector_type(4)));

constexpr int kRows = 64;
constexpr int kUnits = 16;
constexpr int kSc1 = 16;
constexpr unsigned kSpinLimit = 1u << 24;

__device__ __forceinline__ v4f ld4(const float* p) { return *reinterpret_cast<const v4f*>(p); }
__device__ __forceinline__ void st4(float* p, v4f v) { *reinterpret_cast<v4f*>(p) = v; }
__device__ __forceinline__ float sigmoidf_(float x) { return 1.0f / (1.0f + expf(-x)); }
__device__ __forceinline__ float sigmoid_fast(float x) { return __builtin_amdgcn_rcpf(1.0f + __expf(-x)); }
__device__ __forceinline__ float tanh_fast(float x) { return 2.0f * sigmoid_fast(2.0f * x) - 1.0f; }

__device__ __forceinline__ __amdgpu_buffer_rsrc_t rsrc(const float* base) {
  return __builtin_amdgcn_make_buffer_rsrc(const_cast<float*>(base), (short)0, 0x7fffffff, 0x00020000);
}
__device__ __forceinline__ v4f ld4_sc1(__amdgpu_buffer_rsrc_t r, unsigned byte_off) {
  return __builtin_bit_cast(v4f, __builtin_amdgcn_raw_buffer_load_b128(r, (int)byte_off, 0, kSc1));
}
__device__ __forceinline__ void st4_sc1(__amdgpu_buffer_rsrc_t r, unsigned byte_off, v4f v) {
  __builtin_amdgcn_raw_buffer_store_b128(__builtin_bit_cast(v4u, v), r, (int)byte_off, 0, kSc1);
}

__device__ __forceinline__ void spin_gave_up(const GruPArgs& a) {
  atomicAdd(&g_spin_timeouts, 1ull);
  if (a.health) __hip_atomic_store(a.health, 1u, __ATOMIC_RELAXED, __HIP_MEMORY_SCOPE_SYSTEM);
}

__device__ __forceinline__ void wait_count(const GruPArgs& a, unsigned* cnt, unsigned target) {
  if (threadIdx.x == 0) {
    unsigned spins = 0;
    while (__hip_atomic_load(cnt, __ATOMIC_RELAXED, __HIP_MEMORY_SCOPE_AGENT) < target) {
      __builtin_amdgcn_s_sleep(2);
      if (++spins >= a.spin_limit) {
        spin_gave_up(a);
        break;
      }
    }
  }
  __syncthreads();
}

__device__ __forceinline__ void arrive(unsigned* cnt) {
  asm volatile("s_waitcnt vmcnt(0)" ::: "memory");
  __syncthreads();
  if (threadIdx.x == 0) __hip_atomic_fetch_add(cnt, 1u, __ATOMIC_RELAXED, __HIP_MEMORY_SCOPE_AGENT);
}

__device__ __forceinline__ void sync_wait(const GruPArgs& a, unsigned* cnt, int dir, int group, int S, int step,
                                          bool local) {
  if (!a.flags && !local) {
    wait_count(a, cnt, (unsigned)S * step);
    return;
  }
  if (threadIdx.x < 64) {
    unsigned* f = a.counters + pw_flag64(dir, a.G, group, 0);
    const int lane = threadIdx.x;
    unsigned spins = 0;
    while (true) {
      const unsigned v = lane < S ? __hip_atomic_load(f + lane, __ATOMIC_RELAXED, __HIP_MEMORY_SCOPE_AGENT) : 0xffffffffu;
      if (__all(v >= (unsigned)step)) break;
      __builtin_amdgcn_s_sleep(1);
      if (++spins >= a.spin_limit) {
        if (lane == 0) spin_gave_up(a);
        break;
// ... 142 lines not shown
__device__ __forceinline__ void stage_wih(const GruPArgs& a, float* Wx, int dir, int j0, int H) {
  const float* W = a.w_ih + (size_t)dir * 3 * H * a.in;
  for (int v = threadIdx.x; v < 3 * kUnits * kFusedIn; v += 256) {
    const int c = v / kFusedIn, k = v % kFusedIn, g = c / kUnits, jj = c % kUnits;
    Wx[c * kXP + k] = k < a.in ? rnd16<RND>(W[(size_t)(g * H + j0 + jj) * a.in + k]) : 0.f;
  }
}

__device__ __forceinline__ void load_x(const GruPArgs& a, int t, int brow, int lq, float (&xv)[kFusedIn / 4]) {
  const float* xr = a.x_in + ((size_t)brow * a.T + t) * a.in;
#pragma unroll
  for (int m = 0; m < kFusedIn / 4; ++m) {
    const int k = 4 * m + lq;
    xv[m] = (4 * m < a.in && k < a.in) ? xr[k] : 0.f;
  }
}

template <int RND>
__device__ __forceinline__ void fused_gi(const GruPArgs& a, const float* Wx, const float (&xv0)[kFusedIn / 4], int lr,
                                         int lq, float bir, float biz, float bin, float (&gr)[4], float (&gz)[4],
                                         float (&gn)[4]) {
  float xv[kFusedIn / 4];
#pragma unroll
  for (int m = 0; m < kFusedIn / 4; ++m) xv[m] = rnd16<RND>(xv0[m]);
  f32x4 ax[3] = {f32x4{0.f, 0.f, 0.f, 0.f}, f32x4{0.f, 0.f, 0.f, 0.f}, f32x4{0.f, 0.f, 0.f, 0.f}};
#pragma unroll
  for (int m = 0; m < kFusedIn / 4; ++m) {
    if (4 * m >= a.in) break;
#pragma unroll
    for (int g = 0; g < 3; ++g)
      ax[g] = __builtin_amdgcn_mfma_f32_16x16x4f32(xv[m], Wx[(g * kUnits + lr) * kXP + 4 * m + lq], ax[g], 0, 0, 0);
  }
#pragma unroll
  for (int r = 0; r < 4; ++r) {
    gr[r] = ax[0][r] + bir;
    gz[r] = ax[1][r] + biz;
    gn[r] = ax[2][r] + bin;
  }
}

template <int H>
__global__ __launch_bounds__(256, 1) void gru_fwd_persistent_kernel(GruPArgs a) {
  constexpr int WP = H + 4, HTP = kUnits + 4, NKB = H / 16;
  constexpr int RNDX = 0;
  extern __shared__ __attribute__((aligned(16))) float smem[];
  float* Ws = smem;
  float* hT = smem + 3 * kUnits * WP;
  float* Wx = hT + 64 * HTP;
  const int tid = threadIdx.x, lane = tid & 63, wave = tid >> 6, lr = lane & 15, lq = lane >> 4;
  int dir, group, slice;
  bool local;
  place(a, H / kUnits, dir, group, slice, local);
  trace_id(a, dir, group, slice);
  const int T = a.T, j0 = slice * kUnits, j = j0 + lr;
  const int b0 = a.b_begin + group * kRows;
  const int b_last = a.b_end - 1;
  unsigned* cnt = a.counters + pw_counter(dir, a.G, group);

  {
    const float* W = a.w_hh + (size_t)dir * 3 * H * H;
    for (int v = tid; v < 3 * kUnits * H / 4; v += 256) {
      const int c = v / (H / 4), kq = (v % (H / 4)) * 4, g = c / kUnits, jj = c % kUnits;
      st4(Ws + c * WP + kq, ld4(W + (size_t)(g * H + j0 + jj) * H + kq));
    }
  }
  const bool fused = a.x_in != nullptr;
  if (fused) stage_wih<RNDX>(a, Wx, dir, j0, H);
  float xnext[kFusedIn / 4];
  if (fused) load_x(a, dir == 0 ? 0 : a.T - 1, min(a.b_begin + group * kRows + wave * 16 + lr, a.b_end - 1), lq, xnext);
  const float bir = fused ? a.b_ih[dir * 3 * H + j] : 0.f, biz = fused ? a.b_ih[dir * 3 * H + H + j] : 0.f,
              bin = fused ? a.b_ih[dir * 3 * H + 2 * H + j] : 0.f;
  const float bhr = a.b_hh[dir * 3 * H + j], bhz = a.b_hh[dir * 3 * H + H + j], bhn = a.b_hh[dir * 3 * H + 2 * H + j];
  __syncthreads();

  const int B = a.B;
  const int Gp = a.G;
  const __amdgpu_buffer_rsrc_t rx = rsrc(a.xbuf + (size_t)dir * 2 * Gp * 64 * H);
  float hreg[4] = {0.f, 0.f, 0.f, 0.f};
  float gsv[4][4];

  for (int step = 0; step < T; ++step) {
    const int t = dir == 0 ? step : T - 1 - step;
    const int tprev = dir == 0 ? t - 1 : t + 1;
    stamp(a, step, 0);
    float gr[4], gz[4], gn[4];
    if (fused) {
      fused_gi<RNDX>(a, Wx, xnext, lr, lq, bir, biz, bin, gr, gz, gn);
      if (step + 1 < T) load_x(a, dir == 0 ? t + 1 : t - 1, min(b0 + wave * 16 + lr, b_last), lq, xnext);
    } else {
#pragma unroll
      for (int r = 0; r < 4; ++r) {
        const int b = min(b0 + wave * 16 + lq * 4 + r, b_last);
        const float* gi = a.gi + ((size_t)b * T + t) * 6 * H + dir * 3 * H;
        gr[r] = gi[j];
        gz[r] = gi[H + j];
        gn[r] = gi[2 * H + j];
      }
    }
    f32x4 acc[3];
#pragma unroll
    for (int g = 0; g < 3; ++g) acc[g] = f32x4{0.f, 0.f, 0.f, 0.f};
    if (step > 0) {
      sync_wait(a, cnt, dir, group, H / kUnits, step, local);
      stamp(a, step, 1);
      const unsigned base = (unsigned)(((((size_t)((step - 1) & 1) * Gp + group) * 4 + wave) * NKB * 64 + lane) * 16);
      const int rot = slice % NKB;
// ... 20 lines not shown
#pragma unroll
        for (int i = 0; i < 12; ++i) __builtin_amdgcn_sched_group_barrier(0x008, 1, 0);
        __builtin_amdgcn_sched_barrier(0);
      }
      if (a.trace) {
        asm volatile("" ::"v"(acc[0][0]), "v"(acc[1][0]), "v"(acc[2][0]));
        stamp(a, step, 2);
      }
    }
#pragma unroll
    for (int r = 0; r < 4; ++r) {
      const int rl = wave * 16 + lq * 4 + r, b = b0 + rl;
      const float ghn = acc[2][r] + bhn;
      const float rg = sigmoidf_(gr[r] + (acc[0][r] + bhr));
      const float zg = sigmoidf_(gz[r] + (acc[1][r] + bhz));
      const float ng = tanhf(gn[r] + rg * ghn);
      const float h = (1.0f - zg) * ng + zg * hreg[r];
      hreg[r] = h;
      hT[rl * HTP + lr] = h;
      gsv[r][0] = rg;
      gsv[r][1] = zg;
      gsv[r][2] = ng;
      gsv[r][3] = ghn;
    }
    __syncthreads();
    stamp(a, step, 3);
    v4f hv4;
    const int yrl = tid >> 2, yuq = (tid & 3) * 4;
    {
      hv4 = ld4(hT + yrl * HTP + yuq);
      if (step + 1 < T && b0 + yrl <= b_last)
        st4_ho(rx, (unsigned)(((((size_t)(step & 1) * Gp + group) * 4 + (yrl >> 4)) * NKB * 64 + slice * 64 +
                                (yuq >> 2) * 16 + (yrl & 15)) * 16), hv4, local);
    }
    sync_arrive(a, cnt, dir, group, slice, step, local);
    stamp(a, step, 4);
    if (b0 + yrl <= b_last) st4(a.y + ((size_t)(b0 + yrl) * T + t) * 2 * H + dir * H + j0 + yuq, hv4);
    store_gates_il(a, gsv, dir, t, b0 + wave * 16 + lq * 4, b_last, j);
  }
}

template <int H>
__global__ __launch_bounds__(256, 1) void gru_bwd_persistent_kernel(GruPArgs a) {
  constexpr int WP = 3 * H + 4, DTP = kUnits + 4, NKB = 3 * H / 16, CH = 16;
  static_assert(NKB % CH == 0, "chunking");
  extern __shared__ __attribute__((aligned(16))) float smem[];
  float* Wt = smem;
  float* dT = smem + kUnits * WP;
  const int tid = threadIdx.x, lane = tid & 63, wave = tid >> 6, lr = lane & 15, lq = lane >> 4;
  int dir, group, slice;
  bool local;
  place(a, H / kUnits, dir, group, slice, local);
  trace_id(a, dir, group, slice);
  const int T = a.T, B = a.B, j0 = slice * kUnits, j = j0 + lr;
  const int b0 = a.b_begin + group * kRows;
  const int b_last = a.b_end - 1;
  unsigned* cnt = a.counters + pw_counter(dir, a.G, group);

  {
    const float* W = a.w_hh + (size_t)dir * 3 * H * H;
    for (int v = tid; v < 3 * H * kUnits / 4; v += 256) {
      const int c = v / (kUnits / 4), jq = (v % (kUnits / 4)) * 4;
      const v4f w = ld4(W + (size_t)c * H + j0 + jq);
      Wt[(jq + 0) * WP + c] = w.x;
      Wt[(jq + 1) * WP + c] = w.y;
      Wt[(jq + 2) * WP + c] = w.z;
      Wt[(jq + 3) * WP + c] = w.w;
    }
  }
  __syncthreads();

  float* dgh_dir = a.dgh + (size_t)dir * B * T * 3 * H;
  const int Gp = a.G;
  const __amdgpu_buffer_rsrc_t rg_ = rsrc(a.xbuf + (size_t)dir * 2 * Gp * 64 * 3 * H);
  float dhz[4] = {0.f, 0.f, 0.f, 0.f};

  for (int step = 0; step < T; ++step) {
    const int t = dir == 0 ? T - 1 - step : step;
    const int tnext = dir == 0 ? t + 1 : t - 1;
    const int tprev = dir == 0 ? t - 1 : t + 1;
    const bool edge = (step == T - 1);
    stamp(a, step, 0);
    float g_r[4], g_z[4], g_n[4], g_h[4], dyv[4], hpv[4];
#pragma unroll
    for (int r = 0; r < 4; ++r) {
      const int b = min(b0 + wave * 16 + lq * 4 + r, b_last);
      const float* gs = a.gates + (((size_t)dir * T + t) * B + b) * 4 * H;
      const v4f gv = *reinterpret_cast<const v4f*>(gs + 4 * j);
      g_r[r] = gv.x;
      g_z[r] = gv.y;
      g_n[r] = gv.z;
      g_h[r] = gv.w;
      dyv[r] = a.dy[((size_t)b * T + t) * 2 * H + dir * H + j];
      hpv[r] = edge ? 0.f : a.y_in[((size_t)b * T + tprev) * 2 * H + dir * H + j];
    }
    f32x4 acc[2] = {f32x4{0.f, 0.f, 0.f, 0.f}, f32x4{0.f, 0.f, 0.f, 0.f}};
    if (step > 0) {
      sync_wait(a, cnt, dir, group, H / kUnits, step, local);
      stamp(a, step, 1);
      const unsigned base = (unsigned)(((((size_t)((step - 1) & 1) * Gp + group) * 4 + wave) * NKB * 64 + lane) * 16);
      const int rot = (slice * (NKB / (H / kUnits))) % NKB;
      auto kr = [&](int i) { const int v = i + rot; return v >= NKB ? v - NKB : v; };
      v4f dv[2][CH];
#pragma unroll
      for (int kb = 0; kb < CH; ++kb) dv[0][kb] = ld4_sc1(rg_, base + kr(kb) * 1024);
      __builtin_amdgcn_sched_barrier(0);
// ... 100 lines not shown
    if (++spins >= a.spin_limit) {
      if (lane == 0) spin_gave_up(a);
      break;
    }
  }
}

__device__ __forceinline__ void dc_pair_sync(const GruPArgs& a, unsigned* pf, int w, int step) {
  __builtin_amdgcn_fence(__ATOMIC_RELEASE, "workgroup");
  if ((threadIdx.x & 63) == 0) __hip_atomic_store(pf + w, (unsigned)(step + 1), __ATOMIC_RELAXED, __HIP_MEMORY_SCOPE_WORKGROUP);
  unsigned spins = 0;
  while (__hip_atomic_load(pf + (w ^ 1), __ATOMIC_RELAXED, __HIP_MEMORY_SCOPE_WORKGROUP) < (unsigned)(step + 1)) {
    __builtin_amdgcn_s_sleep(0);
    if (++spins >= 4 * a.spin_limit) {
      if ((threadIdx.x & 63) == 0) spin_gave_up(a);
      break;
    }
  }
  __builtin_amdgcn_fence(__ATOMIC_ACQUIRE, "workgroup");
}

__device__ __forceinline__ void dc_flag(const GruPArgs& a, unsigned* f, int step, bool local) {
  asm volatile("s_waitcnt vmcnt(0)" ::: "memory");
  if ((threadIdx.x & 63) == 0) {
    if (local)
      __builtin_amdgcn_raw_buffer_store_b32((unsigned)(step + 1), rsrc(reinterpret_cast<const float*>(f)), 0, 0, 0);
    else
      __hip_atomic_store(f, (unsigned)(step + 1), __ATOMIC_RELAXED, __HIP_MEMORY_SCOPE_AGENT);
  }
}

__device__ __forceinline__ unsigned* dc_flags(const GruPArgs& a, int dir, int group, int c, int rb) {
  return a.counters + pw_flag_dc(dir, a.G, group, c, rb, 0);
}

size_t dc_fwd_lds_floats(int H) { return (size_t)48 * (H + 4) + 16 * 32 * kDcXF + 8 * 128 + 16; }

template <int H, bool FUSED>
__global__ __launch_bounds__(512, 1) void gru_fwd_persistent_dc_kernel(GruPArgs a) {
  constexpr int WP = H + 4, NKB = H / 16, KB2 = NKB / 2;
  static_assert(KB2 == 16, "the k half is 16 k blocks (H = 512)");
  extern __shared__ __attribute__((aligned(16))) float smem[];
  float* Ws = smem;
  float* xch = Ws + 48 * WP;
  float* tp = xch + 16 * 32 * kDcXF;
  unsigned* pf = reinterpret_cast<unsigned*>(tp + 8 * 128);
  const int tid = threadIdx.x, lane = tid & 63, w = __builtin_amdgcn_readfirstlane(tid >> 6);
  const int c = w >> 2, rb = (w >> 1) & 1, kh = w & 1;
  const int lr = lane & 15, lq = lane >> 4;
  int dir, group, slice;
  bool local;
  place(a, H / kUnits, dir, group, slice, local);
  trace_id(a, dir, group, slice);
  const int T = a.T, j0 = slice * kUnits, j = j0 + lr;
  const int rbase = a.b_begin + group * kRows + 32 * c + 16 * rb;
  const int b_last = a.b_end - 1;
  const bool own = (lr >> 3) == kh;

  {
    const float* W = a.w_hh + (size_t)dir * 3 * H * H;
    for (int v = tid; v < 3 * kUnits * H / 4; v += 512) {
      const int cc = v / (H / 4), kq = (v % (H / 4)) * 4, g = cc / kUnits, jj = cc % kUnits;
      st4(Ws + cc * WP + kq, ld4(W + (size_t)(g * H + j0 + jj) * H + kq));
    }
  }
  if (tid < 8) pf[tid] = 0;
  constexpr bool fused = FUSED;
  const int nq = fused ? (a.in + 3) / 4 : 0, mh = (nq + 1) / 2;
  const int m0 = kh ? mh : 0, m1 = kh ? nq : mh;
  constexpr int NX = FUSED ? 8 : 1;
  float wx[3][NX];
#pragma unroll
  for (int g = 0; g < 3; ++g)
#pragma unroll
    for (int i = 0; i < NX; ++i) {
      const int k = 4 * (m0 + i) + lq;
      wx[g][i] = (fused && m0 + i < m1 && k < a.in) ? a.w_ih[((size_t)dir * 3 * H + g * H + j) * a.in + k] : 0.f;
    }
  float xv[NX];
  auto load_xh = [&](int t) {
    const float* xr = a.x_in + ((size_t)min(rbase + lr, b_last) * T + t) * a.in;
#pragma unroll
    for (int i = 0; i < NX; ++i) {
      const int k = 4 * (m0 + i) + lq;
      xv[i] = (m0 + i < m1 && k < a.in) ? xr[k] : 0.f;
    }
  };
  if constexpr (FUSED) load_xh(dir == 0 ? 0 : T - 1);
  const float bir = fused ? a.b_ih[dir * 3 * H + j] : 0.f, biz = fused ? a.b_ih[dir * 3 * H + H + j] : 0.f,
              bin = fused ? a.b_ih[dir * 3 * H + 2 * H + j] : 0.f;
  const float bhr = a.b_hh[dir * 3 * H + j], bhz = a.b_hh[dir * 3 * H + H + j], bhn = a.b_hh[dir * 3 * H + 2 * H + j];
  __syncthreads();
  dc_chain_delay(a, c);

  const int Gp = a.G;
  const __amdgpu_buffer_rsrc_t rx = rsrc(a.xbuf + (size_t)dir * kHandoffSlots * Gp * 64 * H);
  unsigned* myflags = dc_flags(a, dir, group, c, rb);
  const int rot = slice & (KB2 - 1);
  const int slot_id = (lr & 7) + 8 * lq;
  float* mytp = tp + w * 128;
  float hreg[4] = {0.f, 0.f, 0.f, 0.f};

  for (int step = 0; step < T; ++step) {
    const int t = dir == 0 ? step : T - 1 - step;
    stamp(a, step, 0);
    float gr[4], gz[4], gn[4];
// ... 95 lines not shown
        float rg, zg, ng;
        if (a.fast_cell) {
          rg = sigmoid_fast(gr[r] + (acc[0][r] + bhr));
          zg = sigmoid_fast(gz[r] + (acc[1][r] + bhz));
          ng = tanh_fast(gn[r] + rg * ghn);
        } else {
          rg = sigmoidf_(gr[r] + (acc[0][r] + bhr));
          zg = sigmoidf_(gz[r] + (acc[1][r] + bhz));
          ng = tanhf(gn[r] + rg * ghn);
        }
        const float h = (1.0f - zg) * ng + zg * hreg[r];
        hreg[r] = h;
        mytp[(4 * lq + r) * 8 + (lr & 7)] = h;
        gsv[r][0] = rg;
        gsv[r][1] = zg;
        gsv[r][2] = ng;
        gsv[r][3] = ghn;
      }
    }
    dc_wave_lds_fence();
    stamp(a, step, 3);
    const int prow = lane & 15, pq = (lane >> 4) & 1;
    const v4f hv4 = ld4(mytp + prow * 8 + 4 * pq);
    const bool prow_ok = rbase + prow <= b_last;
    if (lane < 32 && step + 1 < T && prow_ok)
      st4_ho(rx, (unsigned)((((((size_t)(step % kHandoffSlots) * Gp + group) * 4 + 2 * c + rb) * NKB + slice) * 64 +
                             32 * kh + lane) * 16), hv4, local);
    dc_flag(a, myflags + 2 * slice + kh, step, local);
    stamp(a, step, 4);
    if (lane < 32 && prow_ok) st4(a.y + ((size_t)(rbase + prow) * T + t) * 2 * H + dir * H + j0 + 8 * kh + 4 * pq, hv4);
    if (own) store_gates_il(a, gsv, dir, t, rbase + 4 * lq, b_last, j);
  }
}


size_t dc_bwd_lds_floats(int H) { return (size_t)16 * (3 * H + 4) + 16 * 32 * 4 + 8 * 512 + 16; }

template <int H>
__global__ __launch_bounds__(512, 1) void gru_bwd_persistent_dc_kernel(GruPArgs a) {
  constexpr int WP = 3 * H + 4, NKB = 3 * H / 16, S = H / kUnits, CH = 8, NCH = 3 * (S / 2) / CH;
  static_assert(S == 32 && NCH * CH == 48, "H = 512");
  extern __shared__ __attribute__((aligned(16))) float smem[];
  float* Wt = smem;
  float* xch = Wt + 16 * WP;
  float* tp = xch + 16 * 32 * 4;
  unsigned* pf = reinterpret_cast<unsigned*>(tp + 8 * 512);
  const int tid = threadIdx.x, lane = tid & 63, w = __builtin_amdgcn_readfirstlane(tid >> 6);
  const int c = w >> 2, rb = (w >> 1) & 1, kh = w & 1;
  const int lr = lane & 15, lq = lane >> 4;
  int dir, group, slice;
  bool local;
  place(a, S, dir, group, slice, local);
  trace_id(a, dir, group, slice);
  const int T = a.T, B = a.B, j0 = slice * kUnits, j = j0 + lr;
  const int rbase = a.b_begin + group * kRows + 32 * c + 16 * rb;
  const int b_last = a.b_end - 1;
  const bool own = (lr >> 3) == kh;

  {
    const float* W = a.w_hh + (size_t)dir * 3 * H * H;
    for (int v = tid; v < 3 * H * kUnits / 4; v += 512) {
      const int cc = v / (kUnits / 4), jq = (v % (kUnits / 4)) * 4;
      const v4f wv = ld4(W + (size_t)cc * H + j0 + jq);
      Wt[(jq + 0) * WP + cc] = wv.x;
      Wt[(jq + 1) * WP + cc] = wv.y;
      Wt[(jq + 2) * WP + cc] = wv.z;
      Wt[(jq + 3) * WP + cc] = wv.w;
    }
  }
  if (tid < 8) pf[tid] = 0;
  __syncthreads();
  dc_chain_delay(a, c);

  float* dgh_dir = a.dgh + (size_t)dir * B * T * 3 * H;
  const int Gp = a.G;
  const __amdgpu_buffer_rsrc_t rg_ = rsrc(a.xbuf + (size_t)dir * kHandoffSlots * Gp * 64 * 3 * H);
  unsigned* myflags = dc_flags(a, dir, group, c, rb);
  const int slot_id = (lr & 7) + 8 * lq;
  float* mytp = tp + w * 512;
  const int rot = slice & 15;
  auto kblock = [&](int i) { const int g = i >> 4; return g * S + 16 * kh + (((i & 15) + rot) & 15); };
  float dhz[4] = {0.f, 0.f, 0.f, 0.f};

  for (int step = 0; step < T; ++step) {
    const int t = dir == 0 ? T - 1 - step : step;
    const int tprev = dir == 0 ? t - 1 : t + 1;
    const bool edge = (step == T - 1);
    stamp(a, step, 0);
    float g_r[4], g_z[4], g_n[4], g_h[4], dyv[4], hpv[4];
#pragma unroll
    for (int r = 0; r < 4; ++r) {
      const int b = min(rbase + lq * 4 + r, b_last);
      const v4f gv = *reinterpret_cast<const v4f*>(a.gates + (((size_t)dir * T + t) * B + b) * 4 * H + 4 * j);
      g_r[r] = gv.x;
      g_z[r] = gv.y;
      g_n[r] = gv.z;
      g_h[r] = gv.w;
      dyv[r] = a.dy[((size_t)b * T + t) * 2 * H + dir * H + j];
      hpv[r] = edge ? 0.f : a.y_in[((size_t)b * T + tprev) * 2 * H + dir * H + j];
    }
    f32x4 acc[2] = {f32x4{0.f, 0.f, 0.f, 0.f}, f32x4{0.f, 0.f, 0.f, 0.f}};
    if (step > 0) {
      dc_wait(a, myflags + 32 * kh, step);
      stamp(a, step, 1);
      dc_stamp_chain1(a, step);
      const unsigned base =
// ... 1244 lines not shown
    const void* k = kernel_ptr<H>(backward, prec);
    const size_t lds = lds_bytes(H, backward, prec);
    SRK_CHECK_HIP(hipFuncSetAttribute(k, hipFuncAttributeMaxDynamicSharedMemorySize, (int)lds));
    SRK_CHECK_HIP(hipOccupancyMaxActiveBlocksPerMultiprocessor(&o, k, 256, lds));
  }
  return (o >= 1 && grid <= cus) ? 1 : 0;
}

}

size_t fwd_lds_bytes(int H) { return (size_t)(3 * 16 * (H + 4) + 64 * 20 + 48 * kXP) * 4; }
size_t bwd_lds_bytes(int H) { return (size_t)(16 * (3 * H + 4) + 64 * 4 * 20) * 4; }

int gru_persistent_groups(int64_t H) {
  if (H != 512) return 0;
  return 4;
}

int gru_persistent_supported(int64_t B, int64_t T, int64_t H, bool backward) {
  const int gmax = gru_persistent_groups(H);
  if (gmax == 0) return 0;
  if ((double)B * T * 3 * H * 4 >= 2147483647.0 || (double)B * T * 2 * H * 4 >= 2147483647.0) return 0;
  const int64_t G = std::min<int64_t>((B + kRows - 1) / kRows, gmax);
  const int grid = (int)(2 * G * (H / kUnits));
  const int prec = matmul_prec();
  int ok = occupancy_ok<512>(backward, prec, grid);
  if (ok > 0 && prec != kPrecF32 && g_opt_gru_lp2) ok = lp2_occupancy_ok<512>(backward, prec);
  return ok < 0 ? 0 : ok;
}

bool lp2_wide(int64_t B, int prec, bool backward, int in_fused) {
  return prec != kPrecF32 && g_opt_gru_lp2 && g_opt_gru_lp_wide && B > 256 && in_fused <= 40 &&
         lp2_occupancy_ok<512>(backward, prec, 4) > 0;
}

int gru_dwhh_fused_parts(int64_t B, int64_t T) {
  const int prec = matmul_prec();
  if (!g_opt_gru_dwhh_fused || prec == kPrecF32 || !g_opt_gru_lp2 || T < 2 || lp2_wide(B, prec, true, 0)) return 0;
  if (lp2_dw_occupancy_ok<512>(prec) <= 0) return 0;
  return (int)((B + 255) / 256) * 8;
}

int gru_bias_part_rows(int64_t B) {
  const int prec = matmul_prec();
  if (lp2_wide(B, prec, true, 0)) return 64;
  return (prec != kPrecF32 && g_opt_gru_lp2) ? kRows2 : kRows;
}

__global__ void __launch_bounds__(256) zero_counters_kernel(unsigned* __restrict__ p, int n) {
  const int i = blockIdx.x * 256 + threadIdx.x;
  if (i < n) __hip_atomic_store(p + i, 0u, __ATOMIC_RELAXED, __HIP_MEMORY_SCOPE_AGENT);
}

int gru_persistent_launch(GruPArgs a, bool backward, hipStream_t s) {
  const int gmax = gru_persistent_groups(a.H);
  SRK_REQUIRE(gmax > 0 && a.H == 512, SRK_ERR_INVALID, "gru persistent: unsupported H");
  const int prec = matmul_prec();
  const bool wide = lp2_wide(a.B, prec, backward, a.x_in ? a.in : 0) && (!backward || a.dgi16 != nullptr);
  const int rows_per_launch = wide ? 512 : gmax * kRows;
  const bool lp2 = prec != kPrecF32 && g_opt_gru_lp2 && (!backward || a.dgi16 != nullptr);
  const int rows_g = wide ? 64 : lp2 ? kRows2 : kRows, slices = lp2 ? a.H / kUnits2 : a.H / kUnits;
  if (lp2 && lp2_occupancy_ok<512>(backward, prec) <= 0)
    SRK_REQUIRE(false, SRK_ERR_INVALID, "gru persistent: the 32 x 32 kernels do not fit one workgroup per CU");
  const bool dc = prec == kPrecF32 && g_opt_gru_dc && dc_occupancy_ok<512>() > 0;
  const bool ow = lp2 && !backward && !wide && g_opt_gru_fwd_worker && a.y16 &&
                  (double)2 * a.T * a.B * 4 * a.H * 4 < 2147483647.0 && lp2_ow_occupancy_ok<512>(prec) > 0;
  for (int c0 = 0; c0 < a.B; c0 += rows_per_launch) {
    GruPArgs ac = a;
    ac.trace = g_opt_gru_trace;
    unsigned* health_host = nullptr;
    if (int rc = health_word(&health_host, &ac.health)) return rc;
    ac.spin_limit = g_opt_gru_spin_limit ? g_opt_gru_spin_limit : kSpinLimit;
    static const int flags_env = [] { const char* v = getenv("SRK_GRU_FLAGS"); return v && *v ? atoi(v) : 0; }();
    ac.flags = flags_env;
    ac.xcd_local = g_opt_gru_xcd_local;
    ac.dc_offset = g_opt_gru_dc_offset;
    ac.fast_cell = g_opt_gru_fast_cell;
    ac.dc_prio = g_opt_gru_dc_prio;
    ac.dw_mode = g_opt_gru_dwhh_fused;
    ac.b_begin = c0;
    ac.b_end = std::min(a.B, c0 + rows_per_launch);
    ac.G = (ac.b_end - c0 + rows_g - 1) / rows_g;
    ac.chunk = c0 / rows_per_launch;
    hipLaunchKernelGGL(zero_counters_kernel, dim3((kCounterFloats + 255) / 256), dim3(256), 0, s, ac.counters,
                       (int)kCounterFloats);
    const dim3 grid((unsigned)(2 * ac.G * slices));
    const double flops = 2.0 * 2.0 * (double)(ac.b_end - c0) * 3 * a.H * a.H * (a.T - 1);
    ProfScope prof(backward ? (prec == kPrecF32 ? "gru_bwd_seq" : "gru_bwd_seq_lp")
                            : (prec == kPrecF32 ? "gru_fwd_seq" : "gru_fwd_seq_lp"), s, flops);
    prof.detail("gru_%s_persistent%s_kernel B%d T%d chunk%d", backward ? "bwd" : "fwd",
                dc ? "_dc" : wide ? "_lp2w" : lp2 ? (backward && ac.dw_part ? "_lp2dw" : ow ? "_lp2ow" : "_lp2") : (prec == kPrecF32 ? "" : "_lp"),
                ac.b_end - c0, a.T, ac.chunk);
    if (dc && backward)
      hipLaunchKernelGGL((gru_bwd_persistent_dc_kernel<512>), grid, dim3(512), dc_bwd_lds_floats(512) * 4, s, ac);
    else if (dc && ac.x_in)
      hipLaunchKernelGGL((gru_fwd_persistent_dc_kernel<512, true>), grid, dim3(512), dc_fwd_lds_floats(512) * 4, s, ac);
    else if (dc)
      hipLaunchKernelGGL((gru_fwd_persistent_dc_kernel<512, false>), grid, dim3(512), dc_fwd_lds_floats(512) * 4, s, ac);
    else if (lp2 && backward && ac.dw_part) {
      SRK_REQUIRE(!wide && ac.y16_in, SRK_ERR_INTERNAL, "gru persistent: fused dW_hh needs the 32-row kernel and y16");
      hipLaunchKernelGGL(reinterpret_cast<void (*)(GruPArgs)>(const_cast<void*>(lp2_dw_kernel_ptr<512>(prec))), grid,
                         dim3(512), lp2_lds_bytes(512, true, 2, true), s, ac);
    } else if (lp2 && !backward && ow) {
      hipLaunchKernelGGL(reinterpret_cast<void (*)(GruPArgs)>(const_cast<void*>(lp2_ow_kernel_ptr<512>(prec))), grid,
                         dim3(512), lp2_lds_bytes(512, false, 2, false, true), s, ac);
    } else if (lp2)
      hipLaunchKernelGGL(reinterpret_cast<void (*)(GruPArgs)>(const_cast<void*>(lp2_kernel_ptr<512>(backward, prec, wide ? 4 : 2))),
                         grid, dim3(wide ? 512 : 256), lp2_lds_bytes(512, backward, wide ? 4 : 2), s, ac);
    else
      hipLaunchKernelGGL(reinterpret_cast<void (*)(GruPArgs)>(const_cast<void*>(kernel_ptr<512>(backward, prec))), grid,
                         dim3(256), lds_bytes(512, backward, prec), s, ac);
    SRK_CHECK_HIP(hipGetLastError());
  }
  return SRK_OK;
}

}

namespace srk {
int health_word(unsigned** host, unsigned** dev) {
  static std::mutex mu;
  static unsigned* h = nullptr;
  static unsigned* d = nullptr;
  std::lock_guard<std::mutex> lk(mu);
  if (!h) {
    void* p = nullptr;
    SRK_CHECK_HIP(hipHostMalloc(&p, 64, hipHostMallocCoherent | hipHostMallocMapped));
    *static_cast<volatile unsigned*>(p) = 0;
    void* dp = nullptr;
    SRK_CHECK_HIP(hipHostGetDevicePointer(&dp, p, 0));
    h = static_cast<unsigned*>(p);
    d = static_cast<unsigned*>(dp);
  }
  *host = h;
  *dev = d;
  return SRK_OK;
}
}

extern "C" int srk_health_check(int sync) {
// ... 73 lines not shown
```

speechrecognitionproject_amd/csrc/runtime.hip:

```cpp
#include <atomic>
#include <functional>
#include <cmath>
#include <cstdarg>
#include <mutex>
#include <vector>

#include "gru_internal.h"
#include "srk_internal.h"

namespace srk {

int g_opt_gru_persistent = 1;
int g_opt_gemm16_kernel = 0;
int g_opt_conv16_sources = 1;
int g_opt_conv_fused_db = 1;
int g_opt_conv_unpool_gather = 1;
int g_opt_conv_tile = 128;
int g_opt_conv_ring = 0x77;
int g_opt_conv_unpool16 = 1;
int g_opt_conv_colsum16 = 1;
int g_opt_conv_ring_qs = 6;
int g_opt_conv_fast16 = 1;
int g_opt_conv_row16 = 1;
int g_opt_conv_row32 = 1;
int g_opt_conv_fw_gemm = 1;
int g_opt_conv_row16_dgrad = 2;
int g_opt_bn_tree = 0;
int g_opt_mfcc_variant = 3;
int g_opt_gemm_streamk = 1;
int g_opt_gemm32_kernel = 0;
static std::atomic<int> g_opt_matmul_prec{kPrecF32};
thread_local int t_prec_override = -1;
int matmul_prec() { return t_prec_override >= 0 ? t_prec_override : g_opt_matmul_prec.load(std::memory_order_relaxed); }
int g_opt_conv_fwd_fp32 = 0;
unsigned long long* g_opt_gru_trace = nullptr;
unsigned g_opt_gru_spin_limit = 0;
int g_opt_gru_xcd_local = 1;
int g_opt_gru_lp2 = 1;
int g_opt_gru_lp_wide = 1;
int g_opt_gru_dc = 1;
unsigned g_opt_gru_dc_offset = 200;
int g_opt_gru_fast_cell = 1;
int g_opt_gru_dc_prio = 0;
int g_opt_gru_dwhh_fused = 1;
int g_opt_gru_fwd_worker = 0;
int g_opt_gru_dwhh_batched = 1;
int g_opt_gemm_skinny = 1;
int g_opt_attn_pool_regs = 1;
std::atomic<int64_t> g_scratch_gen{0};

static thread_local std::string g_last_error;

void set_error(const char* fmt, ...) {
  char buf[1024];
  va_list ap;
  va_start(ap, fmt);
  vsnprintf(buf, sizeof(buf), fmt, ap);
  va_end(ap);
  g_last_error = buf;
}

namespace {

constexpr int kMaxDevices = 64;
DeviceTables g_tables[kMaxDevices];
std::mutex g_mutex;

template <class T>
int upload(T** dst, const std::vector<T>& src) {
  SRK_CHECK_HIP(hipMalloc(reinterpret_cast<void**>(dst), src.size() * sizeof(T)));
  SRK_CHECK_HIP(hipMemcpy(*dst, src.data(), src.size() * sizeof(T), hipMemcpyHostToDevice));
  return SRK_OK;
}

std::vector<double> linspace(double a, double b, int n) {
  std::vector<double> y(n);
  const double step = (b - a) / (n - 1);
  for (int i = 0; i < n; ++i) y[i] = i * step + a;
  y[n - 1] = b;
  return y;
}

std::vector<float2> twiddles(int m, int count) {
  std::vector<float2> t(count);
  for (int k = 0; k < count; ++k) {
    const double a = -2.0 * M_PI * (double)k / (double)m;
    t[k] = make_float2((float)std::cos(a), (float)std::sin(a));
  }
  return t;
}

int to_windows(const std::vector<double>& w, int nf, int nbins, int width, std::vector<int>& lo,
               std::vector<float>& vals) {
  lo.assign(nf, 0);
  vals.assign((size_t)nf * width, 0.f);
  for (int m = 0; m < nf; ++m) {
    int first = -1, last = -1;
    for (int k = 0; k < nbins; ++k)
      if (w[(size_t)m * nbins + k] != 0.0) { if (first < 0) first = k; last = k; }
// ... 349 lines not shown
  }
  if (n == "gru_spin_limit") {
    SRK_REQUIRE(value >= 0 && value <= 0xffffffffLL, SRK_ERR_INVALID, "gru_spin_limit out of range");
    srk::g_opt_gru_spin_limit = (unsigned)value;
    return SRK_OK;
  }
  if (n == "gru_xcd_local") {
    srk::g_opt_gru_xcd_local = value != 0;
    return SRK_OK;
  }
  if (n == "gru_fp32_dual_chain") {
    srk::g_opt_gru_dc = value != 0;
    return SRK_OK;
  }
  if (n == "gru_dc_offset_ns") {
    SRK_REQUIRE(value >= 0 && value <= 1000000, SRK_ERR_INVALID, "gru_dc_offset_ns out of range");
    srk::g_opt_gru_dc_offset = (unsigned)(value / 10);
    return SRK_OK;
  }
  if (n == "gru_fwd_worker") {
    srk::g_opt_gru_fwd_worker = value != 0;
    return SRK_OK;
  }
  if (n == "gru_dwhh_fused") {
    SRK_REQUIRE(value >= 0 && value <= 7, SRK_ERR_INVALID, "gru_dwhh_fused must be 0..7");
    srk::g_opt_gru_dwhh_fused = (value & 1) ? (int)value : 0;
    return SRK_OK;
  }
  if (n == "gru_dc_prio") {
    SRK_REQUIRE(value >= 0 && value <= 2, SRK_ERR_INVALID, "gru_dc_prio must be 0, 1 or 2");
    srk::g_opt_gru_dc_prio = (int)value;
    return SRK_OK;
  }
  if (n == "gru_fp32_fast_cell") {
    srk::g_opt_gru_fast_cell = value != 0;
    return SRK_OK;
  }
  if (n == "gru_lp_wide") {
    srk::g_opt_gru_lp_wide = value != 0;
    return SRK_OK;
  }
  if (n == "gemm_skinny") {
    srk::g_opt_gemm_skinny = value != 0;
    return SRK_OK;
  }
  if (n == "attn_pool_regs") {
    srk::g_opt_attn_pool_regs = value != 0;
    return SRK_OK;
  }
  if (n == "gru_dwhh_batched") {
    srk::g_opt_gru_dwhh_batched = value != 0;
    return SRK_OK;
  }
  if (n == "gru_lp_32x32") {
    srk::g_opt_gru_lp2 = value != 0;
    return SRK_OK;
  }
  if (n == "gru_trace_ptr") {
    srk::g_opt_gru_trace = reinterpret_cast<unsigned long long*>(value);
    return SRK_OK;
  }
  SRK_REQUIRE(false, SRK_ERR_INVALID, "set_option: unknown option '%s'", name);
  SRK_API_END
}

}

extern "C" int64_t srk_scratch_generation(void) { return srk::g_scratch_gen.load(); }
```

speechrecognitionproject_amd/models/model_cnn_bgru.py:

```python
import torch
import torch.nn as nn

from ..nn import BatchNorm1d, BiGRU, Conv1d, Linear, last_step
from ._common import DEVICE, accuracy, class_accuracy


class CNN(nn.Module):
    def __init__(self):
        super().__init__()
        self.conv1 = Conv1d(1, 64, kernel_size=80, stride=4, padding=38, bias=False)
        self.bn1 = BatchNorm1d(64)
        self.conv2 = Conv1d(64, 128, kernel_size=4, stride=2, padding=0, bias=False)
        self.bn2 = BatchNorm1d(128)
        self.conv3 = Conv1d(128, 256, kernel_size=4, stride=2, padding=0, bias=False)
        self.bn3 = BatchNorm1d(256)
        self.conv4 = Conv1d(256, 512, kernel_size=4, stride=2, padding=0, bias=False)
        self.bn4 = BatchNorm1d(512)
        self.fc = Linear(512, 512)

    def forward(self, x):
        x = self.bn1(self.conv1(x), relu=True)
        x = self.bn2(self.conv2(x), relu=True)
        x = self.bn3(self.conv3(x), relu=True)
        x = self.bn4(self.conv4(x), relu=True)
        bs, sl, _ = x.shape
        return self.fc(x.reshape(bs * sl, -1)).view(bs, sl, 512)


class GRU(nn.Module):
    def __init__(self):
        super().__init__()
        self.gru = BiGRU(512, 512, num_layers=2, bidirectional=True, batch_first=True)
        self.fc2 = Linear(512 * 2, 12)

    def forward(self, x):
        x, _ = self.gru(x)
        return self.fc2(last_step(x))


class Network(nn.Module):
    def __init__(self):
        super().__init__()
        self.cnn = CNN()
        self.gru = GRU()

    def forward(self, x):
        if not torch.is_tensor(x):
            x = torch.as_tensor(x)
        x = x.to(DEVICE, torch.float32).reshape(x.shape[0], -1, 1)
        return self.gru(self.cnn(x))
```

speechrecognitionproject_amd/models/model_mfcc_bgru.py:

```python
import torch
import torch.nn as nn

from .. import features
from ..nn import BiGRU, Linear, last_step
from ._common import DEVICE, accuracy, class_accuracy


def compute_mfcc(sample):
    return features.mfcc(sample.reshape(1, -1))[0].cpu()


class Network(nn.Module):

    def __init__(self, num_features=512, num_layers=2, features="mfcc39x51"):
        super().__init__()
        if features not in ("mfcc39x51", "mfcc40x98"):
            raise ValueError("features must be 'mfcc39x51' (the reference) or 'mfcc40x98' (perf-only)")
        self.features = features
        n_in = 39 if features == "mfcc39x51" else 40
        self.gru = BiGRU(n_in, num_features, num_layers=num_layers, bidirectional=True, batch_first=True)
        self.fc = Linear(num_features * 2, 12)

    def forward(self, x):
        with torch.no_grad():
            if self.features == "mfcc39x51":
                inx = features.mfcc(x, time_major=True)
            else:
                inx = features.mfcc40x98(x)
        inx, _ = self.gru(inx)
        return self.fc(last_step(inx))
```

speechrecognitionproject_amd/models/model_mfrn_bgru.py:

```python
import torch
import torch.nn as nn

from .. import features
from ..nn import BatchNorm1d, BiGRU, Conv1d, Linear, last_step
from ._common import DEVICE, accuracy, class_accuracy
from .model_mfcc_bgru import compute_mfcc
from .model_resnet_bgru import BasicBlock, _kaiming


class ResNet(nn.Module):

    def __init__(self, block):
        super().__init__()
        self.inplanes = 64
        self.conv1 = Conv1d(1, 64, kernel_size=640, stride=40, padding=320, bias=False)
        self.bn1 = BatchNorm1d(64)
        self.relu = nn.ReLU(inplace=True)
        self.layer1 = self._make_layer(block, 64, 2)
        self.layer2 = self._make_layer(block, 128, 2, stride=2)
        self.layer3 = self._make_layer(block, 256, 2, stride=2)
        self.layer4 = self._make_layer(block, 512, 2, stride=2)
        self.fc1 = Linear(512, 512)
        for m in self.modules():
            if isinstance(m, Conv1d):
                _kaiming(m)

    def _make_layer(self, block, planes, blocks, stride=1):
        downsample = None
        if stride != 1 or self.inplanes != planes:
            downsample = nn.Sequential(Conv1d(self.inplanes, planes, kernel_size=1, stride=stride, bias=False),
                                       BatchNorm1d(planes))
        layers = [block(self.inplanes, planes, stride, downsample)]
        self.inplanes = planes
        for _ in range(1, blocks):
            layers.append(block(self.inplanes, planes))
        return nn.Sequential(*layers)

    def forward(self, x):
        x = self.bn1(self.conv1(x), relu=True)
        x = self.layer4(self.layer3(self.layer2(self.layer1(x))))
        bs, sl, _ = x.shape
        return self.fc1(x.reshape(bs * sl, -1)).view(bs, sl, 512)


class GRU(nn.Module):
    def __init__(self, num_features=512, num_layers=2):
        super().__init__()
        self.gru = BiGRU(551, num_features, num_layers=num_layers, bidirectional=True, batch_first=True)
        self.fc2 = Linear(num_features * 2, 12)

    def forward(self, x):
        x, _ = self.gru(x)
        return self.fc2(last_step(x))


class Network(nn.Module):
    def __init__(self, num_features=512, num_layers=2):
        super().__init__()
        self.resnet = ResNet(BasicBlock)
        self.gru = GRU(num_features=num_features, num_layers=num_layers)

    def forward(self, x):
        with torch.no_grad():
            mfcc = features.mfcc(x, time_major=True)
        if not torch.is_tensor(x):
            x = torch.as_tensor(x)
        x = x.to(mfcc.device, torch.float32).reshape(x.shape[0], -1, 1)
        r = self.resnet(x)
        return self.gru(torch.cat((r, mfcc), 2))
```

speechrecognitionproject_amd/models/model_resnet_bgru.py:

```python
import torch
import torch.nn as nn

from ..nn import BatchNorm1d, BiGRU, Conv1d, Linear, MaxPool1d, conv1d_nlc, last_step
from ._common import DEVICE, accuracy, class_accuracy


def _kaiming(conv):
    nn.init.kaiming_normal_(conv.weight, mode="fan_out", nonlinearity="relu")


class BasicBlock(nn.Module):
    def __init__(self, inplanes, planes, stride=1, downsample=None):
        super().__init__()
        self.kernel_size, self.padding = 15, 7
        self.conv1 = Conv1d(inplanes, planes, 15, stride=stride, padding=7, bias=False)
        self.bn1 = BatchNorm1d(planes)
        self.conv2 = Conv1d(planes, planes, 15, stride=1, padding=7, bias=False)
        self.bn2 = BatchNorm1d(planes)
        self.downsample = downsample
        self.stride = stride

    def forward(self, x):
        residual = x
        if self.downsample is not None:
            residual = self.downsample[1](self.downsample[0](x))
        out = self.bn1(self.conv1(x), relu=True)
        return self.bn2(self.conv2(out), residual=residual, relu=True)


class ResNet(nn.Module):
    def __init__(self, block, mode):
        super().__init__()
        self.mode = mode
        self.inplanes = 64
        self.dim = 125
        self.conv1 = Conv1d(1, 64, kernel_size=80, stride=16, padding=38, bias=False)
        self.bn1 = BatchNorm1d(64)
        self.relu = nn.ReLU(inplace=True)
        self.layer1 = self._make_layer(block, 64, 2)
        self.layer2 = self._make_layer(block, 128, 2, stride=2)
        self.layer3 = self._make_layer(block, 256, 2, stride=2)
        self.layer4 = self._make_layer(block, 512, 2, stride=2)
        self.fc1 = Linear(512, 512)
        self.backend_conv1 = nn.Sequential(
            Conv1d(self.dim, 2 * self.dim, 5, stride=2, padding=0, bias=False), BatchNorm1d(2 * self.dim), nn.ReLU(True),
            MaxPool1d(2),
            Conv1d(2 * self.dim, 4 * self.dim, 5, stride=2, padding=0, bias=False), BatchNorm1d(4 * self.dim),
            nn.ReLU(True))
        self.backend_conv2 = nn.Sequential(
            Linear(4 * self.dim, self.dim), BatchNorm1d(self.dim), nn.ReLU(True), Linear(self.dim, 12))
        for m in self.modules():
            if isinstance(m, (Conv1d, nn.Conv1d)):
                _kaiming(m)

    def _make_layer(self, block, planes, blocks, stride=1):
        downsample = None
        if stride != 1 or self.inplanes != planes:
            downsample = nn.Sequential(Conv1d(self.inplanes, planes, kernel_size=1, stride=stride, bias=False),
                                       BatchNorm1d(planes))
        layers = [block(self.inplanes, planes, stride, downsample)]
        self.inplanes = planes
        for _ in range(1, blocks):
            layers.append(block(self.inplanes, planes))
        return nn.Sequential(*layers)

    def forward(self, x):
        x = self.bn1(self.conv1(x), relu=True)
        x = self.layer4(self.layer3(self.layer2(self.layer1(x))))
        bs, sl, _ = x.shape
        x = self.fc1(x.reshape(bs * sl, -1))
        if self.mode == 1:
            x = x.view(bs, sl, 512).transpose(1, 2).contiguous()
            conv_a, bn_a, _, pool, conv_b, bn_b, _ = self.backend_conv1
            pa = (-conv_a.out_channels) % 4
            wa = torch.cat([conv_a.weight, conv_a.weight.new_zeros((pa,) + tuple(conv_a.weight.shape[1:]))])
            wb = torch.cat([conv_b.weight, conv_b.weight.new_zeros((conv_b.out_channels, pa, conv_b.kernel_size[0]))], 1)
            x = bn_a.forward_padded(conv1d_nlc(x, wa, None, conv_a.stride[0]), relu=True)
            x = bn_b(conv1d_nlc(pool(x), wb, None, conv_b.stride[0]), relu=True)
            fc_a, bn_h, _, fc_b = self.backend_conv2
            return fc_b(bn_h(fc_a(x.mean(1)), relu=True))
        return x.view(bs, sl, 512)


class GRU(nn.Module):
    def __init__(self, num_features=512, num_layers=2):
        super().__init__()
        self.gru = BiGRU(512, num_features, num_layers=num_layers, bidirectional=True, batch_first=True)
        self.fc2 = Linear(num_features * 2, 12)

    def forward(self, x):
        x, _ = self.gru(x)
        return self.fc2(last_step(x))


class Network(nn.Module):
    def __init__(self, num_features=512, num_layers=2, mode=0):
        super().__init__()
        self.mode = mode
        self.resnet = ResNet(BasicBlock, mode=mode)
        self.gru = GRU(num_features=num_features, num_layers=num_layers)

    def forward(self, x):
        if not torch.is_tensor(x):
            x = torch.as_tensor(x)
        x = x.to(DEVICE, torch.float32).reshape(x.shape[0], -1, 1)
        x = self.resnet(x)
        if self.mode != 1:
            x = self.gru(x)
        return x
```

speechrecognitionproject_amd/models/model_spec_bgru.py:

```python
import torch
import torch.nn as nn

from .. import features
from ..nn import BiGRU, Linear, last_step
from ._common import DEVICE, accuracy, class_accuracy


def compute_spec(sample):
    return features.spec(sample.reshape(1, -1))[0].cpu()


class Network(nn.Module):
    def __init__(self, num_features=512, num_layers=2):
        super().__init__()
        self.gru = BiGRU(321, num_features, num_layers=num_layers, bidirectional=True, batch_first=True)
        self.fc = Linear(num_features * 2, 12)

    def forward(self, x):
        with torch.no_grad():
            inx = features.spec(x, transposed=True)
        inx, _ = self.gru(inx)
        return self.fc(last_step(inx))
```

speechrecognitionproject_amd/nn.py:

```python
import ctypes
import math
import os

import torch
import torch.nn as tnn

from . import _lib
from ._lib import call
from .features import ptr, require_gpu, stream_ptr


def _optr(t):
    return None if t is None else ptr(t)


def _check_cuda(*ts):
    for t in ts:
        if t is not None and (t.device.type != "cuda" or t.dtype != torch.float32):
            raise _lib.SrkError("libsrk ops need float32 CUDA tensors, got %s %s" % (t.device, t.dtype))


def _adjacent(a, b):
    return (a.is_contiguous() and b.is_contiguous() and a.dtype == b.dtype and a.shape == b.shape
            and a.untyped_storage().data_ptr() == b.untyped_storage().data_ptr()
# ... 39 lines not shown
        w_ih, w_hh = _dir_pair(w_ih_f, w_ih_r), _dir_pair(w_hh_f, w_hh_r)
        b_ih, b_hh = _dir_pair(b_ih_f, b_ih_r), _dir_pair(b_hh_f, b_hh_r)
        _check_cuda(x, w_ih, w_hh, b_ih, b_hh)
        y = torch.empty((B, T, 2 * H), device=x.device, dtype=torch.float32)
        ws = torch.empty(int(_lib.lib().srk_gru_workspace_floats(B, T, IN, H, 0)), device=x.device)
        x16 = _copy16_get(x) if IN % 8 == 0 else None
        call("srk_gru_layer_fwd_x16", ptr(x), _optr(x16), B, T, IN, H, ptr(w_ih),
             ptr(w_hh), ptr(b_ih), ptr(b_hh), ptr(y), ptr(ws), stream_ptr())
        ctx.x16 = x16
        off = int(_lib.lib().srk_gru_y16_offset(B, T, IN, H)) if _copy16_wanted(2 * H) else -1
        if off >= 0 and grad_on and any(ctx.needs_input_grad):
            _copy16_put(y, ws[off:].view(torch.int16)[:y.numel()])
        ctx.save_for_backward(x, w_ih, w_hh, y, ws)
        ctx.dims = (B, T, IN, H)
        ctx.params = (w_ih_f, w_ih_r, w_hh_f, w_hh_r, b_ih_f, b_ih_r, b_hh_f, b_hh_r)
        ctx.prec = _lib.matmul_precision()
        red = _reducer_of(w_ih_f)
        if red is not None and grad_on and any(ctx.needs_input_grad):
            red.persistent_pending(1)
        return y

    @staticmethod
    def backward(ctx, dy):
        x, w_ih, w_hh, y, ws = ctx.saved_tensors
        B, T, IN, H = ctx.dims
        P = ctx.params
        dy = dy.contiguous()
        dx = torch.empty_like(x) if ctx.needs_input_grad[0] else None
        targets = [_grad_pair(P[2 * i], P[2 * i + 1]) for i in range(4)]
        acc = all(t is not None for t in targets) and all(ctx.needs_input_grad[2:])
        if acc:
            dw_ih, dw_hh, db_ih, db_hh = targets
        else:
            dw_ih, dw_hh = torch.empty_like(w_ih), torch.empty_like(w_hh)
            db_ih = torch.empty((2, 3 * H), device=x.device)
            db_hh = torch.empty((2, 3 * H), device=x.device)
        ws2 = torch.empty(int(_lib.lib().srk_gru_workspace_floats(B, T, IN, H, 1)), device=x.device)
        _copy16_drop(y)
        x16, ctx.x16 = ctx.x16, None
        with _lib.precision_scope(ctx.prec):
            call("srk_gru_layer_bwd_x16", ptr(x), _optr(x16), B, T, IN, H, ptr(w_ih),
                 ptr(w_hh), ptr(y), ptr(ws), ptr(dy), _optr(dx), ptr(dw_ih), ptr(dw_hh),
                 ptr(db_ih), ptr(db_hh), int(acc), ptr(ws2), stream_ptr())
        red = _reducer_of(P[0])
        if red is not None:
            red.persistent_done()
            if acc:
                red.mark_ready(P)
        if acc:
            return (dx, None) + (None,) * 8
        return (dx, None, dw_ih[0], dw_ih[1], dw_hh[0], dw_hh[1], db_ih[0], db_ih[1], db_hh[0], db_hh[1])


class BiGRU(tnn.Module):

    def __init__(self, input_size, hidden_size, num_layers=1, bidirectional=True, batch_first=True):
        super().__init__()
        if not (bidirectional and batch_first):
            raise ValueError("BiGRU implements bidirectional=True, batch_first=True (the reference's config)")
        self.input_size, self.hidden_size, self.num_layers = input_size, hidden_size, num_layers
        self.bidirectional, self.batch_first = True, True
        H = hidden_size
        k = 1.0 / H ** 0.5
        for layer in range(num_layers):
            inp = input_size if layer == 0 else 2 * H
            for sfx in ("", "_reverse"):
                for name, shape in (("weight_ih", (3 * H, inp)), ("weight_hh", (3 * H, H)),
                                    ("bias_ih", (3 * H,)), ("bias_hh", (3 * H,))):
                    p = tnn.Parameter(torch.empty(shape).uniform_(-k, k))
                    setattr(self, "%s_l%d%s" % (name, layer, sfx), p)
            for name in ("weight_ih", "weight_hh", "bias_ih", "bias_hh"):
                getattr(self, "%s_l%d" % (name, layer))._srk_pair = getattr(self, "%s_l%d_reverse" % (name, layer))

    def _pairs(self, layer):
        return [getattr(self, "%s_l%d%s" % (name, layer, sfx))
                for name in ("weight_ih", "weight_hh", "bias_ih", "bias_hh") for sfx in ("", "_reverse")]

    def forward(self, x):
        require_gpu()
        h = x
        finals = []
        for layer in range(self.num_layers):
            h = _GRULayerFn.apply(h, torch.is_grad_enabled(), *self._pairs(layer))
            H = self.hidden_size
            finals += [h[:, -1, :H], h[:, 0, H:]]
        return h, torch.stack(finals)


class _LastStepFn(torch.autograd.Function):

    @staticmethod
    def forward(ctx, x):
        ctx.T = x.shape[1]
        return x[:, -1, :]

    @staticmethod
    def backward(ctx, g):
        return tnn.functional.pad(g.unsqueeze(1), (0, 0, ctx.T - 1, 0))


def last_step(x):
    return _LastStepFn.apply(x)


class _AttentionPoolFn(torch.autograd.Function):

    @staticmethod
    def forward(ctx, y, q, scale):
        y, q = y.contiguous(), q.contiguous()
        _check_cuda(y, q)
        if y.dim() != 3 or q.shape != (y.shape[0], y.shape[2]):
            raise _lib.SrkError("attention pool: y must be [B, T, D] and q [B, D], got %s and %s"
                                % (tuple(y.shape), tuple(q.shape)))
        B, T, D = y.shape
        out = torch.empty((B, D), device=y.device)
        alpha = torch.empty((B, T), device=y.device)
        call("srk_attn_pool_fwd", ptr(y), ptr(q), B, T, D, scale, ptr(out), ptr(alpha), stream_ptr())
        ctx.save_for_backward(y, q, alpha)
        ctx.scale = scale
        ctx.mark_non_differentiable(alpha)
        return out, alpha

    @staticmethod
    def backward(ctx, dctx, _dalpha):
        y, q, alpha = ctx.saved_tensors
        B, T, D = y.shape
        dctx = dctx.contiguous()
        dy, dq = torch.empty_like(y), torch.empty_like(q)
        call("srk_attn_pool_bwd", ptr(y), ptr(q), ptr(alpha), ptr(dctx), B, T, D, ctx.scale, ptr(dy), ptr(dq),
             stream_ptr())
        return dy, dq, None


class AttentionPool(tnn.Module):

    def __init__(self, scale=None):
        super().__init__()
        self.scale = scale

# ... 886 lines not shown
```

Before: 51740 utt/s.

## Compute only the last timestep of the top BiGRU layer's reverse direction

Adds a top-layer BiGRU path that returns only the final timestep. The reverse direction at t=T-1 needs just one cell step from a zero state, so it is computed with a single skinny GEMM and an elementwise kernel. The persistent recurrence then runs only the forward direction, and the full reverse input projection and recurrence are skipped. The backward pass builds the padded gradient internally and handles the single reverse cell separately. The change also adds a GEMM plan_batch/no_split hint and brings in a new mode option with default 3, at the cost of much new code and the risk of divergence from the full layer's gradients.

New measurement: 55250 utt/s (median of 6 runs). 1.07x the previous value.

```diff
diff --git a/include/srk.h b/include/srk.h
--- a/include/srk.h
+++ b/include/srk.h
@@ -100,6 +100,14 @@
                           const float* w_ih, const float* w_hh, const float* y, const float* ws_fwd, const float* dy,
                           float* dx, float* dw_ih, float* dw_hh, float* db_ih, float* db_hh, int accumulate,
                           float* ws, void* stream);
+int64_t srk_gru_top_last_workspace_floats(int64_t B, int64_t T, int64_t in, int64_t H, int backward);
+int srk_gru_top_last_fwd(const float* x, const void* x16, int64_t B, int64_t T, int64_t in, int64_t H,
+                         const float* w_ih, const float* w_hh, const float* b_ih, const float* b_hh, float* y,
+                         float* y_last, float* ws, int* mode, void* stream);
+int srk_gru_top_last_bwd(const float* x, const void* x16, int64_t B, int64_t T, int64_t in, int64_t H,
+                         const float* w_ih, const float* w_hh, const float* y, const float* ws_fwd,
+                         const float* dy_last, int mode, float* dx, float* dw_ih, float* dw_hh, float* db_ih,
+                         float* db_hh, int accumulate, float* ws, void* stream);
 
 int64_t srk_conv2d_workspace_floats(int64_t Ci, int64_t Co, int64_t KH, int64_t KW);
 int srk_conv2d_nhwc_fwd(const float* x, int64_t N, int64_t H, int64_t W, int64_t Ci, const float* w,
diff --git a/speechrecognitionproject_amd/_lib.py b/speechrecognitionproject_amd/_lib.py
--- a/speechrecognitionproject_amd/_lib.py
+++ b/speechrecognitionproject_amd/_lib.py
@@ -61,6 +61,9 @@
     "srk_gru_y16_offset": [_I64, _I64, _I64, _I64],
     "srk_gru_layer_fwd_x16": [_P, _P, _I64, _I64, _I64, _I64, _P, _P, _P, _P, _P, _P, _P],
     "srk_gru_layer_bwd_x16": [_P, _P, _I64, _I64, _I64, _I64, _P, _P, _P, _P, _P, _P, _P, _P, _P, _P, _I, _P, _P],
+    "srk_gru_top_last_workspace_floats": [_I64, _I64, _I64, _I64, _I],
+    "srk_gru_top_last_fwd": [_P, _P, _I64, _I64, _I64, _I64, _P, _P, _P, _P, _P, _P, _P, _P, _P],
+    "srk_gru_top_last_bwd": [_P, _P, _I64, _I64, _I64, _I64, _P, _P, _P, _P, _P, _I, _P, _P, _P, _P, _P, _I, _P, _P],
     "srk_conv2d_workspace_floats": [_I64, _I64, _I64, _I64],
     "srk_conv2d_nhwc_fwd": [_P, _I64, _I64, _I64, _I64, _P, _P, _I64, _I64, _I64, _I64, _I64, _I64, _I64, _P, _P,
                             _P],
@@ -124,6 +127,7 @@
     "srk_avgpool_nhwc_bwd": [_P, _I64, _I64, _I64, _P, _P],
 }
 _RESTYPE = {"srk_last_error": ctypes.c_char_p, "srk_spin_timeouts": ctypes.c_int64, "srk_scratch_generation": ctypes.c_int64, "srk_gru_workspace_floats": ctypes.c_int64, "srk_gru_y16_offset": ctypes.c_int64,
+            "srk_gru_top_last_workspace_floats": ctypes.c_int64,
             "srk_conv2d_workspace_floats": ctypes.c_int64, "srk_conv1_pool_workspace_floats": ctypes.c_int64,
             "srk_pitch_workspace_bytes": ctypes.c_int64, "srk_source_stamp": ctypes.c_char_p,
             "srk_pcen_workspace_floats": ctypes.c_int64, "srk_dwconv2d_workspace_floats": ctypes.c_int64}
diff --git a/speechrecognitionproject_amd/csrc/gemm.h b/speechrecognitionproject_amd/csrc/gemm.h
--- a/speechrecognitionproject_amd/csrc/gemm.h
+++ b/speechrecognitionproject_amd/csrc/gemm.h
@@ -16,6 +16,8 @@
   int prec = -1;
   const uint16_t* A16 = nullptr;
   const uint16_t* B16 = nullptr;
+  bool no_split = false;
+  int plan_batch = 0;
 };
 
 int gemm_f32(const GemmDesc& d, hipStream_t stream);
diff --git a/speechrecognitionproject_amd/csrc/gemm.hip b/speechrecognitionproject_amd/csrc/gemm.hip
--- a/speechrecognitionproject_amd/csrc/gemm.hip
+++ b/speechrecognitionproject_amd/csrc/gemm.hip
@@ -1161,7 +1161,7 @@
 }
 
 int skinny_kind(const GemmDesc& d) {
-  if (!g_opt_gemm_skinny || d.batch != 1 || d.A16 || d.B16 || d.K <= 0) return -1;
+  if (!g_opt_gemm_skinny || d.batch != 1 || d.plan_batch > 1 || d.A16 || d.B16 || d.K <= 0) return -1;
   if (d.N <= 16 && !d.ta && d.M <= 65535 * 16 && d.M * d.K <= (int64_t)1 << 24) return 0;
   if (d.M <= 16 && !d.tb && d.K <= 1024 && d.N * d.K <= (int64_t)1 << 24) return 1;
   if (d.K <= 16 && !d.tb && d.M <= 65535 && d.M * d.N <= (int64_t)1 << 24) return 2;
@@ -1552,8 +1552,9 @@
   ka.group_m = group_env > 0 ? group_env
                              : std::max(1, (int)std::lround(std::sqrt(32.0 * per_cu * BN / (double)BM)));
   ka.remap = remap;
-  const bool can_split = allow_split && (d.batch == 1 || split_batched);
-  int splits = can_split ? choose_splits(tm * tn * d.batch, d.K, BK, slots, 16) : 1;
+  const int pb = std::max(d.batch, d.plan_batch);
+  const bool can_split = allow_split && !d.no_split && (pb == 1 || split_batched);
+  int splits = can_split ? choose_splits(tm * tn * pb, d.K, BK, slots, 16) : 1;
   static const int splits_env = env_int("SRK_GEMM_SPLITS", 0);
   if (splits_env > 0 && d.batch == 1 && d.K >= (int64_t)splits_env * 4 * BK) splits = splits_env;
   ka.kchunk = splits > 1 ? ((d.K + splits - 1) / splits + BK - 1) / BK * BK : std::max<int64_t>(d.K, 1);
@@ -1710,9 +1711,10 @@
 int launch_p32(const GemmDesc& d, hipStream_t s) {
   KernelArgs ka;
   int splits = 1;
-  const int64_t tiles = ((d.M + 255) / 256) * ((d.N + 255) / 256) * d.batch;
+  const int pb = std::max(d.batch, d.plan_batch);
+  const int64_t tiles = ((d.M + 255) / 256) * ((d.N + 255) / 256) * pb;
   const int64_t ki = (d.K + kP32BK - 1) / kP32BK;
-  const bool streamk = g_opt_gemm_streamk && d.batch == 1 && !d.rowsum && tiles < kCUs && tiles * 2 >= kCUs && ki >= 32;
+  const bool streamk = g_opt_gemm_streamk && pb == 1 && !d.no_split && !d.rowsum && tiles < kCUs && tiles * 2 >= kCUs && ki >= 32;
   if (int rc = plan_launch(d, 256, 256, kP32BK, 1, ka, &splits, !streamk && tiles * 2 < kCUs, true)) return rc;
   if (streamk) {
     ka.sk_wgs = kCUs;
@@ -1736,7 +1738,7 @@
   const double ext_a = (double)(d.ta ? d.K : d.M) * d.lda * 4, ext_b = (double)(d.tb ? d.N : d.K) * d.ldb * 4;
   const bool p32_ok = vec && ext_a < 2147483000.0 && ext_b < 2147483000.0;
   const int kern32 = g_opt_gemm32_kernel ? g_opt_gemm32_kernel
-                                         : (!TB && ((d.M >= 2048 && d.N >= 1024) || d.batch > 1) ? 2 : 1);
+                                         : (!TB && ((d.M >= 2048 && d.N >= 1024) || d.batch > 1 || d.plan_batch > 1) ? 2 : 1);
   SRK_REQUIRE(!d.rowsum || d.batch == 1 || (p32_ok && kern32 == 2), SRK_ERR_INVALID,
               "gemm: batched row sums need the fp32 ping-pong kernel (16-B operand rows)");
   if (p32_ok && kern32 == 2) return launch_p32<TA, TB>(d, s);
diff --git a/speechrecognitionproject_amd/csrc/gru.hip b/speechrecognitionproject_amd/csrc/gru.hip
--- a/speechrecognitionproject_amd/csrc/gru.hip
+++ b/speechrecognitionproject_amd/csrc/gru.hip
@@ -27,8 +27,6 @@
   float* dgh_edge;
   float* dhz;
 };
-
-__device__ __forceinline__ float sigmoidf_(float x) { return 1.0f / (1.0f + expf(-x)); }
 
 typedef float v4f __attribute__((ext_vector_type(4)));
 __device__ __forceinline__ v4f ld4(const float* p) { return *reinterpret_cast<const v4f*>(p); }
@@ -256,6 +254,79 @@
   }
 }
 
+__global__ void gather_last_kernel(const float* __restrict__ y, int64_t B, int T, int C, float* __restrict__ y_last) {
+  const int64_t i = (int64_t)blockIdx.x * blockDim.x + threadIdx.x;
+  if (i >= B * C) return;
+  const int64_t b = i / C;
+  y_last[i] = y[(b * T + T - 1) * C + (i - b * C)];
+}
+__global__ void pad_last_kernel(const float* __restrict__ dy_last, int64_t B, int T, int C, float* __restrict__ dy) {
+  const int64_t i = (int64_t)blockIdx.x * blockDim.x + threadIdx.x, c4 = C / 4;
+  if (i >= B * T * c4) return;
+  const int64_t row = i / c4, b = row / T;
+  const int c = (int)(i - row * c4) * 4;
+  v4f v = v4f{0.f, 0.f, 0.f, 0.f};
+  if (row - b * T == T - 1) {
+    const float* s = dy_last + b * C + c;
+    v = v4f{s[0], s[1], s[2], s[3]};
+  }
+  st4(dy + i * 4, v);
+}
+__global__ void zero_cols_kernel(float* __restrict__ X, int64_t rows, int cols, int c0, int ld) {
+  const int64_t i = (int64_t)blockIdx.x * blockDim.x + threadIdx.x, c4 = cols / 4;
+  if (i >= rows * c4) return;
+  const int64_t r = i / c4;
+  st4(X + r * ld + c0 + (i - r * c4) * 4, v4f{0.f, 0.f, 0.f, 0.f});
+}
+template <bool FAST>
+__global__ void rev_cell_fwd_kernel(const float* __restrict__ gi, const float* __restrict__ b_hh, int64_t B, int T,
+                                    int H, float* __restrict__ y, float* __restrict__ y_last,
+                                    float* __restrict__ gates) {
+  const int64_t i = (int64_t)blockIdx.x * blockDim.x + threadIdx.x;
+  if (i >= B * H) return;
+  const int64_t b = i / H, row = b * T + T - 1;
+  const int j = (int)(i - b * H);
+  const float* g = gi + row * 6 * H + 3 * H;
+  const float bhr = b_hh[3 * H + j], bhz = b_hh[4 * H + j], ghn = b_hh[5 * H + j];
+  float rg, zg, ng;
+  if (FAST) {
+    rg = sigmoid_fast(g[j] + bhr);
+    zg = sigmoid_fast(g[H + j] + bhz);
+    ng = tanh_fast(g[2 * H + j] + rg * ghn);
+  } else {
+    rg = sigmoidf_(g[j] + bhr);
+    zg = sigmoidf_(g[H + j] + bhz);
+    ng = tanhf(g[2 * H + j] + rg * ghn);
+  }
+  const float h = (1.0f - zg) * ng;
+  y[row * 2 * H + H + j] = h;
+  y_last[b * 2 * H + H + j] = h;
+  y_last[b * 2 * H + j] = y[row * 2 * H + j];
+  st4(gates + (((int64_t)T + T - 1) * B + b) * 4 * H + 4 * j, v4f{rg, zg, ng, ghn});
+}
+__global__ void rev_cell_bwd_kernel(const float* __restrict__ gates, const float* __restrict__ dy_last, int64_t B, int T,
+                                    int H, float* __restrict__ dgi, float* __restrict__ dgh_edge) {
+  const int64_t i = (int64_t)blockIdx.x * blockDim.x + threadIdx.x;
+  if (i >= B * H) return;
+  const int64_t b = i / H;
+  const int j = (int)(i - b * H);
+  const v4f gv = ld4(gates + (((int64_t)T + T - 1) * B + b) * 4 * H + 4 * j);
+  const float rg = gv.x, zg = gv.y, ng = gv.z, ghn = gv.w;
+  const float dh = dy_last[b * 2 * H + H + j];
+  const float dn = dh * (1.0f - zg);
+  const float daz = dh * (0.f - ng) * zg * (1.0f - zg);
+  const float dan = dn * (1.0f - ng * ng);
+  const float dar = dan * ghn * rg * (1.0f - rg);
+  float* d = dgi + (b * T + T - 1) * 6 * H + 3 * H;
+  d[j] = dar;
+  d[H + j] = daz;
+  d[2 * H + j] = dan;
+  float* e = dgh_edge + (B + b) * 3 * H;
+  e[j] = dar;
+  e[H + j] = daz;
+  e[2 * H + j] = dan * rg;
+}
+
 int check_dims(int64_t B, int64_t T, int64_t in, int64_t H) {
   SRK_REQUIRE(B > 0 && T > 0 && in > 0 && H > 0, SRK_ERR_INVALID, "gru: dims must be positive");
   SRK_REQUIRE(H % kBK == 0, SRK_ERR_INVALID, "gru: hidden size must be a multiple of 128");
@@ -476,13 +547,19 @@
   return pad_end(B, T, in, H, 0) + up64(BT * in8 / 2 + 1) + up64(6 * H * in8 / 2 + 1);
 }
 
-int srk_gru_layer_fwd_x16(const float* x, const void* x16_in, int64_t B, int64_t T, int64_t in, int64_t H,
-                          const float* w_ih, const float* w_hh, const float* b_ih, const float* b_hh, float* y,
-                          float* ws, void* stream) {
-  SRK_API_BEGIN
-  if (int rc = srk::check_dims(B, T, in, H)) return rc;
-  SRK_REQUIRE(x && w_ih && w_hh && b_ih && b_hh && y && ws, SRK_ERR_INVALID, "gru_fwd: null pointer");
-  hipStream_t s = srk::as_stream(stream);
+static bool persistent_pair(int64_t B, int64_t T, int64_t H) {
+  return srk::g_opt_gru_persistent && srk::gru_persistent_supported(B, T, H, false) &&
+         srk::gru_persistent_supported(B, T, H, true);
+}
+static bool top_last_path(int64_t B, int64_t T, int64_t H) {
+  return srk::matmul_prec() == srk::kPrecF32 && H == 512 && persistent_pair(B, T, H);
+}
+static int top_last_mode(int64_t B, int64_t T, int64_t H) { return top_last_path(B, T, H) ? srk::g_opt_gru_top_last : 0; }
+
+static int layer_fwd(const float* x, const void* x16_in, int64_t B, int64_t T, int64_t in, int64_t H,
+                     const float* w_ih, const float* w_hh, const float* b_ih, const float* b_hh, float* y,
+                     float* ws, int top_last, float* y_last, hipStream_t s) {
+  const bool rev_cell = top_last >= 2;
   float* gi = ws;
   float* gates = ws + B * T * 6 * H;
   uint16_t* y16 = nullptr;
@@ -526,16 +603,26 @@
     xa = xp;
     wa = wp;
   }
-  const bool persistent = srk::g_opt_gru_persistent && srk::gru_persistent_supported(B, T, H, false) &&
-                          srk::gru_persistent_supported(B, T, H, true);
+  const bool persistent = persistent_pair(B, T, H);
+  SRK_REQUIRE(!rev_cell || (persistent && y_last), SRK_ERR_INTERNAL, "gru_fwd: rev_cell off the persistent path");
   const bool fuse = persistent && in <= srk::kFusedIn;
   if (!fuse) {
     GemmDesc g;
-    g.M = B * T; g.N = 6 * H; g.K = ink;
+    g.M = B * T; g.N = rev_cell ? 3 * H : 6 * H; g.K = ink;
     g.A = xa; g.lda = ink;
     g.B = wa; g.ldb = ink; g.tb = true;
     g.C = gi; g.ldc = 6 * H;
     g.bias = b_ih; g.bias_mode = 1;
+    if (int rc = srk::gemm_f32(g, s)) return rc;
+  }
+  if (rev_cell) {
+    GemmDesc g;
+    g.M = B; g.N = 3 * H; g.K = ink;
+    g.A = xa + (T - 1) * ink; g.lda = T * ink;
+    g.B = wa + 3 * H * ink; g.ldb = ink; g.tb = true;
+    g.C = gi + (T - 1) * 6 * H + 3 * H; g.ldc = T * 6 * H;
+    g.bias = b_ih + 3 * H; g.bias_mode = 1;
+    g.no_split = top_last == 3;
     if (int rc = srk::gemm_f32(g, s)) return rc;
   }
   if (persistent) {
@@ -545,7 +632,19 @@
     if (fuse) { p.x_in = x; p.w_ih = w_ih; p.b_ih = b_ih; p.in = (int)in; }
     p.xbuf = ws + fwd_xbuf_off(B, T, H);
     p.counters = reinterpret_cast<unsigned*>(ws + fwd_counter_off(B, T, H));
-    return srk::gru_persistent_launch(p, false, s);
+    p.one_dir = rev_cell ? 1 : 0;
+    if (int rc = srk::gru_persistent_launch(p, false, s)) return rc;
+    if (rev_cell) {
+      const dim3 grid((unsigned)((B * H + 255) / 256));
+      if (srk::gru_fp32_fast_cell())
+        hipLaunchKernelGGL(srk::rev_cell_fwd_kernel<true>, grid, dim3(256), 0, s, gi, b_hh, B, (int)T, (int)H, y,
+                           y_last, gates);
+      else
+        hipLaunchKernelGGL(srk::rev_cell_fwd_kernel<false>, grid, dim3(256), 0, s, gi, b_hh, B, (int)T, (int)H, y,
+                           y_last, gates);
+      SRK_CHECK_HIP(hipGetLastError());
+    }
+    return SRK_OK;
   }
   srk::GruArgs a{};
   a.B = (int)B; a.T = (int)T; a.H = (int)H; a.in = (int)in;
@@ -559,6 +658,39 @@
   }
   SRK_CHECK_HIP(hipGetLastError());
   return SRK_OK;
+}
+
+int srk_gru_layer_fwd_x16(const float* x, const void* x16_in, int64_t B, int64_t T, int64_t in, int64_t H,
+                          const float* w_ih, const float* w_hh, const float* b_ih, const float* b_hh, float* y,
+                          float* ws, void* stream) {
+  SRK_API_BEGIN
+  if (int rc = srk::check_dims(B, T, in, H)) return rc;
+  SRK_REQUIRE(x && w_ih && w_hh && b_ih && b_hh && y && ws, SRK_ERR_INVALID, "gru_fwd: null pointer");
+  return layer_fwd(x, x16_in, B, T, in, H, w_ih, w_hh, b_ih, b_hh, y, ws, 0, nullptr, srk::as_stream(stream));
+  SRK_API_END
+}
+
+int64_t srk_gru_top_last_workspace_floats(int64_t B, int64_t T, int64_t in, int64_t H, int backward) {
+  return srk_gru_workspace_floats(B, T, in, H, backward) + (backward ? up64(B * T * 2 * H) : 0);
+}
+
+int srk_gru_top_last_fwd(const float* x, const void* x16_in, int64_t B, int64_t T, int64_t in, int64_t H,
+                         const float* w_ih, const float* w_hh, const float* b_ih, const float* b_hh, float* y,
+                         float* y_last, float* ws, int* mode, void* stream) {
+  SRK_API_BEGIN
+  if (int rc = srk::check_dims(B, T, in, H)) return rc;
+  SRK_REQUIRE(x && w_ih && w_hh && b_ih && b_hh && y && y_last && ws && mode, SRK_ERR_INVALID,
+              "gru_top_last_fwd: null pointer");
+  hipStream_t s = srk::as_stream(stream);
+  *mode = top_last_mode(B, T, H);
+  if (int rc = layer_fwd(x, x16_in, B, T, in, H, w_ih, w_hh, b_ih, b_hh, y, ws, *mode, y_last, s)) return rc;
+  if (*mode < 2) {
+    const int64_t n = B * 2 * H;
+    hipLaunchKernelGGL(srk::gather_last_kernel, dim3((unsigned)((n + 255) / 256)), dim3(256), 0, s, y, B, (int)T,
+                       (int)(2 * H), y_last);
+    SRK_CHECK_HIP(hipGetLastError());
+  }
+  return SRK_OK;
   SRK_API_END
 }
 
@@ -570,15 +702,10 @@
                                accumulate, ws, stream);
 }
 
-int srk_gru_layer_bwd_x16(const float* x, const void* x16_in, int64_t B, int64_t T, int64_t in, int64_t H,
-                          const float* w_ih, const float* w_hh, const float* y, const float* ws_fwd, const float* dy,
-                          float* dx, float* dw_ih, float* dw_hh, float* db_ih, float* db_hh, int accumulate,
-                          float* ws, void* stream) {
-  SRK_API_BEGIN
-  if (int rc = srk::check_dims(B, T, in, H)) return rc;
-  SRK_REQUIRE(x && w_ih && w_hh && y && ws_fwd && dy && dw_ih && dw_hh && db_ih && db_hh && ws, SRK_ERR_INVALID,
-              "gru_bwd: null pointer");
-  hipStream_t s = srk::as_stream(stream);
+static int layer_bwd(const float* x, const void* x16_in, int64_t B, int64_t T, int64_t in, int64_t H,
+                     const float* w_ih, const float* w_hh, const float* y, const float* ws_fwd, const float* dy,
+                     const float* dy_last, int top_last, float* dx, float* dw_ih, float* dw_hh, float* db_ih,
+                     float* db_hh, int accumulate, float* ws, hipStream_t s) {
   const int64_t BT = B * T;
   if (use_h16(B, T, in, H)) {
     const int64_t in8 = in8_of(in);
@@ -681,14 +808,27 @@
   a.dy = dy; a.dgi = dgi; a.dgh = dgh; a.dgh_edge = dgh_edge; a.dhz = dhz;
   a.G = (int)((B + srk::kRows - 1) / srk::kRows);
   a.S = (int)(H / srk::kUnits);
-  if (srk::g_opt_gru_persistent && srk::gru_persistent_supported(B, T, H, false) &&
-      srk::gru_persistent_supported(B, T, H, true)) {
+  const bool persistent = persistent_pair(B, T, H);
+  SRK_REQUIRE(!top_last || (persistent && dy_last), SRK_ERR_INTERNAL, "gru_bwd: top_last off the persistent path");
+  if (persistent) {
     srk::GruPArgs p{};
     p.B = (int)B; p.T = (int)T; p.H = (int)H;
     p.w_hh = w_hh; p.y_in = y; p.gates = a.gates; p.dy = dy; p.dgi = dgi; p.dgh = dgh; p.dgh_edge = dgh_edge;
     p.xbuf = ws + bwd_xbuf_off(B, T, H);
     p.counters = reinterpret_cast<unsigned*>(ws + bwd_counter_off(B, T, H));
+    p.one_dir = top_last >= 2 ? 1 : 0;
     if (int rc = srk::gru_persistent_launch(p, true, s)) return rc;
+    if (top_last == 3) {
+      const int64_t n4 = BT * 3 * H / 4;
+      hipLaunchKernelGGL(srk::zero_cols_kernel, dim3((unsigned)((n4 + 255) / 256)), dim3(256), 0, s, dgi, BT,
+                         (int)(3 * H), (int)(3 * H), (int)(6 * H));
+      SRK_CHECK_HIP(hipGetLastError());
+    }
+    if (top_last >= 2) {
+      hipLaunchKernelGGL(srk::rev_cell_bwd_kernel, dim3((unsigned)((B * H + 255) / 256)), dim3(256), 0, s, a.gates,
+                         dy_last, B, (int)T, (int)H, dgi, dgh_edge);
+      SRK_CHECK_HIP(hipGetLastError());
+    }
   } else {
   const dim3 grid((unsigned)(2 * a.G * a.S));
   for (int step = 0; step < T; ++step) {
@@ -705,14 +845,24 @@
   float* wpad = pad ? ws + pad_off(B, T, H, 1) : nullptr;
   float* dwpad = pad ? wpad + 6 * H * in4 : nullptr;
   float* dxpad = pad ? dwpad + 6 * H * in4 : nullptr;
+  const bool rev_last = top_last == 1 || top_last == 2;
+  const float* dgi_rev = dgi + (T - 1) * 6 * H + 3 * H;
   {
     GemmDesc g;
-    g.M = 6 * H; g.N = pad ? in4 : in; g.K = BT;
+    g.M = rev_last ? 3 * H : 6 * H; g.N = pad ? in4 : in; g.K = BT;
     g.A = dgi; g.lda = 6 * H; g.ta = true;
     g.B = pad ? ws_fwd + pad_off(B, T, H, 0) : x; g.ldb = pad ? in4 : in;
     g.C = pad ? dwpad : dw_ih; g.ldc = pad ? in4 : in; g.beta = pad ? 0.f : beta;
     g.rowsum = db_ih; g.rowsum_beta = beta;
     if ((rc = srk::gemm_f32(g, s))) return rc;
+    if (rev_last) {
+      g.K = B;
+      g.A = dgi_rev; g.lda = T * 6 * H;
+      g.B += (T - 1) * g.ldb; g.ldb *= T;
+      g.C += 3 * H * g.ldc;
+      g.rowsum = db_ih + 3 * H;
+      if ((rc = srk::gemm_f32(g, s))) return rc;
+    }
     if (pad) {
       const int64_t n = 6 * H * in;
       hipLaunchKernelGGL(srk::unpad_cols_kernel, dim3((unsigned)((n + 255) / 256)), dim3(256), 0, s, dwpad, 6 * H,
@@ -730,7 +880,20 @@
     g.rowsum = db_hh; g.rowsum_beta = beta;
     g.batch = 2; g.sA = BT * 3 * H - 3 * H; g.sB = 3 * H; g.sC = 3 * H * H; g.sRS = 3 * H;
     const bool batched = srk::g_opt_gru_dwhh_batched && srk::gemm_f32_batched_rowsum_ok(g);
-    if (g.K > 0 && batched) {
+    if (top_last) {
+      g.batch = 1;
+      g.plan_batch = (top_last == 3 && batched) ? 2 : 0;
+      if (g.K > 0) {
+        if ((rc = srk::gemm_f32(g, s))) return rc;
+      } else if (!accumulate) {
+        SRK_CHECK_HIP(hipMemsetAsync(dw_hh, 0, sizeof(float) * 3 * H * H, s));
+        SRK_CHECK_HIP(hipMemsetAsync(db_hh, 0, sizeof(float) * 3 * H, s));
+      }
+      if (!accumulate) {
+        SRK_CHECK_HIP(hipMemsetAsync(dw_hh + 3 * H * H, 0, sizeof(float) * 3 * H * H, s));
+        SRK_CHECK_HIP(hipMemsetAsync(db_hh + 3 * H, 0, sizeof(float) * 3 * H, s));
+      }
+    } else if (g.K > 0 && batched) {
       if ((rc = srk::gemm_f32(g, s))) return rc;
     } else if (g.K > 0) {
       g.batch = 1;
@@ -746,12 +909,20 @@
   }
   if (dx) {
     GemmDesc g;
-    g.M = BT; g.N = pad ? in4 : in; g.K = 6 * H;
+    g.M = BT; g.N = pad ? in4 : in; g.K = rev_last ? 3 * H : 6 * H;
     g.A = dgi; g.lda = 6 * H;
     if (pad && (rc = srk::pad_cols(w_ih, 6 * H, in, wpad, s))) return rc;
     g.B = pad ? wpad : w_ih; g.ldb = pad ? in4 : in;
     g.C = pad ? dxpad : dx; g.ldc = pad ? in4 : in;
     if ((rc = srk::gemm_f32(g, s))) return rc;
+    if (rev_last) {
+      g.M = B;
+      g.A = dgi_rev; g.lda = T * 6 * H;
+      g.B += 3 * H * g.ldb;
+      g.C += (T - 1) * g.ldc; g.ldc *= T;
+      g.beta = 1.f;
+      if ((rc = srk::gemm_f32(g, s))) return rc;
+    }
     if (pad) {
       const int64_t n = BT * in;
       hipLaunchKernelGGL(srk::unpad_cols_kernel, dim3((unsigned)((n + 255) / 256)), dim3(256), 0, s, dxpad, BT,
@@ -760,7 +931,41 @@
     }
   }
   return SRK_OK;
+}
+
+int srk_gru_layer_bwd_x16(const float* x, const void* x16_in, int64_t B, int64_t T, int64_t in, int64_t H,
+                          const float* w_ih, const float* w_hh, const float* y, const float* ws_fwd, const float* dy,
+                          float* dx, float* dw_ih, float* dw_hh, float* db_ih, float* db_hh, int accumulate,
+                          float* ws, void* stream) {
+  SRK_API_BEGIN
+  if (int rc = srk::check_dims(B, T, in, H)) return rc;
+  SRK_REQUIRE(x && w_ih && w_hh && y && ws_fwd && dy && dw_ih && dw_hh && db_ih && db_hh && ws, SRK_ERR_INVALID,
+              "gru_bwd: null pointer");
+  return layer_bwd(x, x16_in, B, T, in, H, w_ih, w_hh, y, ws_fwd, dy, nullptr, 0, dx, dw_ih, dw_hh, db_ih, db_hh,
+                   accumulate, ws, srk::as_stream(stream));
   SRK_API_END
 }
 
-}
+int srk_gru_top_last_bwd(const float* x, const void* x16_in, int64_t B, int64_t T, int64_t in, int64_t H,
+                         const float* w_ih, const float* w_hh, const float* y, const float* ws_fwd,
+                         const float* dy_last, int mode, float* dx, float* dw_ih, float* dw_hh, float* db_ih,
+                         float* db_hh, int accumulate, float* ws, void* stream) {
+  SRK_API_BEGIN
+  if (int rc = srk::check_dims(B, T, in, H)) return rc;
+  SRK_REQUIRE(x && w_ih && w_hh && y && ws_fwd && dy_last && dw_ih && dw_hh && db_ih && db_hh && ws, SRK_ERR_INVALID,
+              "gru_top_last_bwd: null pointer");
+  SRK_REQUIRE(mode >= 0 && mode <= 3, SRK_ERR_INVALID, "gru_top_last_bwd: mode must be the forward's (0 .. 3)");
+  SRK_REQUIRE(mode == 0 || top_last_path(B, T, H), SRK_ERR_INVALID,
+              "gru_top_last_bwd: mode %d needs the fp32 persistent path its forward ran on", mode);
+  hipStream_t s = srk::as_stream(stream);
+  float* dy = ws + srk_gru_workspace_floats(B, T, in, H, 1);
+  const int64_t n4 = B * T * 2 * H / 4;
+  hipLaunchKernelGGL(srk::pad_last_kernel, dim3((unsigned)((n4 + 255) / 256)), dim3(256), 0, s, dy_last, B, (int)T,
+                     (int)(2 * H), dy);
+  SRK_CHECK_HIP(hipGetLastError());
+  return layer_bwd(x, x16_in, B, T, in, H, w_ih, w_hh, y, ws_fwd, dy, dy_last, mode, dx, dw_ih, dw_hh, db_ih, db_hh,
+                   accumulate, ws, s);
+  SRK_API_END
+}
+
+}
diff --git a/speechrecognitionproject_amd/csrc/gru_internal.h b/speechrecognitionproject_amd/csrc/gru_internal.h
--- a/speechrecognitionproject_amd/csrc/gru_internal.h
+++ b/speechrecognitionproject_amd/csrc/gru_internal.h
@@ -52,12 +52,18 @@
   const uint16_t* y16_in;
   float* dw_part;
   int dw_mode;
+  int one_dir;
 };
+
+__device__ __forceinline__ float sigmoidf_(float x) { return 1.0f / (1.0f + expf(-x)); }
+__device__ __forceinline__ float sigmoid_fast(float x) { return __builtin_amdgcn_rcpf(1.0f + __expf(-x)); }
+__device__ __forceinline__ float tanh_fast(float x) { return 2.0f * sigmoid_fast(2.0f * x) - 1.0f; }
 
 size_t fwd_lds_bytes(int H);
 size_t bwd_lds_bytes(int H);
 int gru_persistent_supported(int64_t B, int64_t T, int64_t H, bool backward);
 int gru_persistent_launch(GruPArgs a, bool backward, hipStream_t s);
+int gru_fp32_fast_cell();
 
 extern int g_opt_gru_persistent;
 extern unsigned long long* g_opt_gru_trace;
@@ -73,6 +79,7 @@
 int gru_dwhh_fused_parts(int64_t B, int64_t T);
 extern int g_opt_gru_dwhh_fused;
 extern int g_opt_gru_fwd_worker;
+extern int g_opt_gru_top_last;
 int health_word(unsigned** host, unsigned** dev);
 
 }
diff --git a/speechrecognitionproject_amd/csrc/gru_persistent.hip b/speechrecognitionproject_amd/csrc/gru_persistent.hip
--- a/speechrecognitionproject_amd/csrc/gru_persistent.hip
+++ b/speechrecognitionproject_amd/csrc/gru_persistent.hip
@@ -22,9 +22,6 @@
 
 __device__ __forceinline__ v4f ld4(const float* p) { return *reinterpret_cast<const v4f*>(p); }
 __device__ __forceinline__ void st4(float* p, v4f v) { *reinterpret_cast<v4f*>(p) = v; }
-__device__ __forceinline__ float sigmoidf_(float x) { return 1.0f / (1.0f + expf(-x)); }
-__device__ __forceinline__ float sigmoid_fast(float x) { return __builtin_amdgcn_rcpf(1.0f + __expf(-x)); }
-__device__ __forceinline__ float tanh_fast(float x) { return 2.0f * sigmoid_fast(2.0f * x) - 1.0f; }
 
 __device__ __forceinline__ __amdgpu_buffer_rsrc_t rsrc(const float* base) {
   return __builtin_amdgcn_make_buffer_rsrc(const_cast<float*>(base), (short)0, 0x7fffffff, 0x00020000);
@@ -273,6 +270,7 @@
   bool local;
   place(a, H / kUnits, dir, group, slice, local);
   trace_id(a, dir, group, slice);
+  if (a.one_dir && dir == 1) return;
   const int T = a.T, j0 = slice * kUnits, j = j0 + lr;
   const int b0 = a.b_begin + group * kRows;
   const int b_last = a.b_end - 1;
@@ -399,6 +397,7 @@
   bool local;
   place(a, H / kUnits, dir, group, slice, local);
   trace_id(a, dir, group, slice);
+  if (a.one_dir && dir == 1) return;
   const int T = a.T, B = a.B, j0 = slice * kUnits, j = j0 + lr;
   const int b0 = a.b_begin + group * kRows;
   const int b_last = a.b_end - 1;
@@ -605,6 +604,7 @@
   bool local;
   place(a, H / kUnits, dir, group, slice, local);
   trace_id(a, dir, group, slice);
+  if (a.one_dir && dir == 1) return;
   const int T = a.T, j0 = slice * kUnits, j = j0 + lr;
   const int rbase = a.b_begin + group * kRows + 32 * c + 16 * rb;
   const int b_last = a.b_end - 1;
@@ -806,6 +806,7 @@
   bool local;
   place(a, S, dir, group, slice, local);
   trace_id(a, dir, group, slice);
+  if (a.one_dir && dir == 1) return;
   const int T = a.T, B = a.B, j0 = slice * kUnits, j = j0 + lr;
   const int rbase = a.b_begin + group * kRows + 32 * c + 16 * rb;
   const int b_last = a.b_end - 1;
@@ -2156,10 +2157,13 @@
   if (i < n) __hip_atomic_store(p + i, 0u, __ATOMIC_RELAXED, __HIP_MEMORY_SCOPE_AGENT);
 }
 
+int gru_fp32_fast_cell() { return g_opt_gru_fast_cell && g_opt_gru_dc && dc_occupancy_ok<512>() > 0; }
+
 int gru_persistent_launch(GruPArgs a, bool backward, hipStream_t s) {
   const int gmax = gru_persistent_groups(a.H);
   SRK_REQUIRE(gmax > 0 && a.H == 512, SRK_ERR_INVALID, "gru persistent: unsupported H");
   const int prec = matmul_prec();
+  SRK_REQUIRE(!a.one_dir || prec == kPrecF32, SRK_ERR_INVALID, "gru persistent: one_dir is an fp32 mode");
   const bool wide = lp2_wide(a.B, prec, backward, a.x_in ? a.in : 0) && (!backward || a.dgi16 != nullptr);
   const int rows_per_launch = wide ? 512 : gmax * kRows;
   const bool lp2 = prec != kPrecF32 && g_opt_gru_lp2 && (!backward || a.dgi16 != nullptr);
@@ -2189,7 +2193,7 @@
     hipLaunchKernelGGL(zero_counters_kernel, dim3((kCounterFloats + 255) / 256), dim3(256), 0, s, ac.counters,
                        (int)kCounterFloats);
     const dim3 grid((unsigned)(2 * ac.G * slices));
-    const double flops = 2.0 * 2.0 * (double)(ac.b_end - c0) * 3 * a.H * a.H * (a.T - 1);
+    const double flops = 2.0 * (a.one_dir ? 1.0 : 2.0) * (double)(ac.b_end - c0) * 3 * a.H * a.H * (a.T - 1);
     ProfScope prof(backward ? (prec == kPrecF32 ? "gru_bwd_seq" : "gru_bwd_seq_lp")
                             : (prec == kPrecF32 ? "gru_fwd_seq" : "gru_fwd_seq_lp"), s, flops);
     prof.detail("gru_%s_persistent%s_kernel B%d T%d chunk%d", backward ? "bwd" : "fwd",
diff --git a/speechrecognitionproject_amd/csrc/runtime.hip b/speechrecognitionproject_amd/csrc/runtime.hip
--- a/speechrecognitionproject_amd/csrc/runtime.hip
+++ b/speechrecognitionproject_amd/csrc/runtime.hip
@@ -45,6 +45,7 @@
 int g_opt_gru_dwhh_fused = 1;
 int g_opt_gru_fwd_worker = 0;
 int g_opt_gru_dwhh_batched = 1;
+int g_opt_gru_top_last = 3;
 int g_opt_gemm_skinny = 1;
 int g_opt_attn_pool_regs = 1;
 std::atomic<int64_t> g_scratch_gen{0};
@@ -500,6 +501,11 @@
     srk::g_opt_gru_dwhh_batched = value != 0;
     return SRK_OK;
   }
+  if (n == "gru_top_last") {
+    SRK_REQUIRE(value >= 0 && value <= 3, SRK_ERR_INVALID, "gru_top_last must be 0 .. 3");
+    srk::g_opt_gru_top_last = (int)value;
+    return SRK_OK;
+  }
   if (n == "gru_lp_32x32") {
     srk::g_opt_gru_lp2 = value != 0;
     return SRK_OK;
diff --git a/speechrecognitionproject_amd/models/model_cnn_bgru.py b/speechrecognitionproject_amd/models/model_cnn_bgru.py
--- a/speechrecognitionproject_amd/models/model_cnn_bgru.py
+++ b/speechrecognitionproject_amd/models/model_cnn_bgru.py
@@ -1,7 +1,7 @@
 import torch
 import torch.nn as nn
 
-from ..nn import BatchNorm1d, BiGRU, Conv1d, Linear, last_step
+from ..nn import BatchNorm1d, BiGRU, Conv1d, Linear
 from ._common import DEVICE, accuracy, class_accuracy
 
 
@@ -34,8 +34,7 @@
         self.fc2 = Linear(512 * 2, 12)
 
     def forward(self, x):
-        x, _ = self.gru(x)
-        return self.fc2(last_step(x))
+        return self.fc2(self.gru.forward_last(x))
 
 
 class Network(nn.Module):
diff --git a/speechrecognitionproject_amd/models/model_mfcc_bgru.py b/speechrecognitionproject_amd/models/model_mfcc_bgru.py
--- a/speechrecognitionproject_amd/models/model_mfcc_bgru.py
+++ b/speechrecognitionproject_amd/models/model_mfcc_bgru.py
@@ -2,7 +2,7 @@
 import torch.nn as nn
 
 from .. import features
-from ..nn import BiGRU, Linear, last_step
+from ..nn import BiGRU, Linear
 from ._common import DEVICE, accuracy, class_accuracy
 
 
@@ -27,5 +27,4 @@
                 inx = features.mfcc(x, time_major=True)
             else:
                 inx = features.mfcc40x98(x)
-        inx, _ = self.gru(inx)
-        return self.fc(last_step(inx))
+        return self.fc(self.gru.forward_last(inx))
diff --git a/speechrecognitionproject_amd/models/model_mfrn_bgru.py b/speechrecognitionproject_amd/models/model_mfrn_bgru.py
--- a/speechrecognitionproject_amd/models/model_mfrn_bgru.py
+++ b/speechrecognitionproject_amd/models/model_mfrn_bgru.py
@@ -2,7 +2,7 @@
 import torch.nn as nn
 
 from .. import features
-from ..nn import BatchNorm1d, BiGRU, Conv1d, Linear, last_step
+from ..nn import BatchNorm1d, BiGRU, Conv1d, Linear
 from ._common import DEVICE, accuracy, class_accuracy
 from .model_mfcc_bgru import compute_mfcc
 from .model_resnet_bgru import BasicBlock, _kaiming
@@ -50,8 +50,7 @@
         self.fc2 = Linear(num_features * 2, 12)
 
     def forward(self, x):
-        x, _ = self.gru(x)
-        return self.fc2(last_step(x))
+        return self.fc2(self.gru.forward_last(x))
 
 
 class Network(nn.Module):
diff --git a/speechrecognitionproject_amd/models/model_resnet_bgru.py b/speechrecognitionproject_amd/models/model_resnet_bgru.py
--- a/speechrecognitionproject_amd/models/model_resnet_bgru.py
+++ b/speechrecognitionproject_amd/models/model_resnet_bgru.py
@@ -1,7 +1,7 @@
 import torch
 import torch.nn as nn
 
-from ..nn import BatchNorm1d, BiGRU, Conv1d, Linear, MaxPool1d, conv1d_nlc, last_step
+from ..nn import BatchNorm1d, BiGRU, Conv1d, Linear, MaxPool1d, conv1d_nlc
 from ._common import DEVICE, accuracy, class_accuracy
 
 
@@ -89,8 +89,7 @@
         self.fc2 = Linear(num_features * 2, 12)
 
     def forward(self, x):
-        x, _ = self.gru(x)
-        return self.fc2(last_step(x))
+        return self.fc2(self.gru.forward_last(x))
 
 
 class Network(nn.Module):
diff --git a/speechrecognitionproject_amd/models/model_spec_bgru.py b/speechrecognitionproject_amd/models/model_spec_bgru.py
--- a/speechrecognitionproject_amd/models/model_spec_bgru.py
+++ b/speechrecognitionproject_amd/models/model_spec_bgru.py
@@ -2,7 +2,7 @@
 import torch.nn as nn
 
 from .. import features
-from ..nn import BiGRU, Linear, last_step
+from ..nn import BiGRU, Linear
 from ._common import DEVICE, accuracy, class_accuracy
 
 
@@ -19,5 +19,4 @@
     def forward(self, x):
         with torch.no_grad():
             inx = features.spec(x, transposed=True)
-        inx, _ = self.gru(inx)
-        return self.fc(last_step(inx))
+        return self.fc(self.gru.forward_last(inx))
diff --git a/speechrecognitionproject_amd/nn.py b/speechrecognitionproject_amd/nn.py
--- a/speechrecognitionproject_amd/nn.py
+++ b/speechrecognitionproject_amd/nn.py
@@ -115,6 +115,65 @@
         return (dx, None, dw_ih[0], dw_ih[1], dw_hh[0], dw_hh[1], db_ih[0], db_ih[1], db_hh[0], db_hh[1])
 
 
+class _GRUTopLastFn(torch.autograd.Function):
+
+    @staticmethod
+    def forward(ctx, x, grad_on, w_ih_f, w_ih_r, w_hh_f, w_hh_r, b_ih_f, b_ih_r, b_hh_f, b_hh_r):
+        B, T, IN = x.shape
+        H = w_hh_f.shape[-1]
+        x = x.contiguous()
+        w_ih, w_hh = _dir_pair(w_ih_f, w_ih_r), _dir_pair(w_hh_f, w_hh_r)
+        b_ih, b_hh = _dir_pair(b_ih_f, b_ih_r), _dir_pair(b_hh_f, b_hh_r)
+        _check_cuda(x, w_ih, w_hh, b_ih, b_hh)
+        y = torch.empty((B, T, 2 * H), device=x.device, dtype=torch.float32)
+        y_last = torch.empty((B, 2 * H), device=x.device, dtype=torch.float32)
+        ws = torch.empty(int(_lib.lib().srk_gru_top_last_workspace_floats(B, T, IN, H, 0)), device=x.device)
+        x16 = _copy16_get(x) if IN % 8 == 0 else None
+        mode = ctypes.c_int(0)
+        call("srk_gru_top_last_fwd", ptr(x), _optr(x16), B, T, IN, H, ptr(w_ih), ptr(w_hh), ptr(b_ih), ptr(b_hh),
+             ptr(y), ptr(y_last), ptr(ws), ctypes.byref(mode), stream_ptr())
+        ctx.x16 = x16
+        ctx.mode = mode.value
+        ctx.save_for_backward(x, w_ih, w_hh, y, ws)
+        ctx.dims = (B, T, IN, H)
+        ctx.params = (w_ih_f, w_ih_r, w_hh_f, w_hh_r, b_ih_f, b_ih_r, b_hh_f, b_hh_r)
+        ctx.prec = _lib.matmul_precision()
+        red = _reducer_of(w_ih_f)
+        if red is not None and grad_on and any(ctx.needs_input_grad):
+            red.persistent_pending(1)
+        return y_last
+
+    @staticmethod
+    def backward(ctx, dy_last):
+        x, w_ih, w_hh, y, ws = ctx.saved_tensors
+        B, T, IN, H = ctx.dims
+        P = ctx.params
+        dy_last = dy_last.contiguous()
+        dx = torch.empty_like(x) if ctx.needs_input_grad[0] else None
+        targets = [_grad_pair(P[2 * i], P[2 * i + 1]) for i in range(4)]
+        acc = all(t is not None for t in targets) and all(ctx.needs_input_grad[2:])
+        if acc:
+            dw_ih, dw_hh, db_ih, db_hh = targets
+        else:
+            dw_ih, dw_hh = torch.empty_like(w_ih), torch.empty_like(w_hh)
+            db_ih = torch.empty((2, 3 * H), device=x.device)
+            db_hh = torch.empty((2, 3 * H), device=x.device)
+        ws2 = torch.empty(int(_lib.lib().srk_gru_top_last_workspace_floats(B, T, IN, H, 1)), device=x.device)
+        x16, ctx.x16 = ctx.x16, None
+        with _lib.precision_scope(ctx.prec):
+            call("srk_gru_top_last_bwd", ptr(x), _optr(x16), B, T, IN, H, ptr(w_ih), ptr(w_hh), ptr(y), ptr(ws),
+                 ptr(dy_last), ctx.mode, _optr(dx), ptr(dw_ih), ptr(dw_hh), ptr(db_ih), ptr(db_hh), int(acc), ptr(ws2),
+                 stream_ptr())
+        red = _reducer_of(P[0])
+        if red is not None:
+            red.persistent_done()
+            if acc:
+                red.mark_ready(P)
+        if acc:
+            return (dx, None) + (None,) * 8
+        return (dx, None, dw_ih[0], dw_ih[1], dw_hh[0], dw_hh[1], db_ih[0], db_ih[1], db_hh[0], db_hh[1])
+
+
 class BiGRU(tnn.Module):
 
     def __init__(self, input_size, hidden_size, num_layers=1, bidirectional=True, batch_first=True):
@@ -148,6 +207,13 @@
             H = self.hidden_size
             finals += [h[:, -1, :H], h[:, 0, H:]]
         return h, torch.stack(finals)
+
+    def forward_last(self, x):
+        require_gpu()
+        h = x
+        for layer in range(self.num_layers - 1):
+            h = _GRULayerFn.apply(h, torch.is_grad_enabled(), *self._pairs(layer))
+        return _GRUTopLastFn.apply(h, torch.is_grad_enabled(), *self._pairs(self.num_layers - 1))
 
 
 class _LastStepFn(torch.autograd.Function):
```
